# wengflow/robust-e-nerf

Hardware: AMD Instinct MI355X
Metric: train_rays_per_sec (higher is better)
Workload: dtype f32; 1 GPU; BASELINE configs[1]: synthetic ficus-like event stream, 65536 events/step/GPU = 2 renders x 65536 rays x 128 samples, arch ngp, fp32, l_diff (2 renders), fwd+bwd+Adam; sampler=uniform; sampler=uniform, samples_per_ray=128, parallelism=dp1, front_prefetched=False, mlp_precision=highest, device_counts=False, device_count_overflows=0, fwd_chunks=8, dist_world_size=1

## Files before the change

### include/ren_amd.h

```cpp
#ifndef REN_AMD_H
#define REN_AMD_H

#include <stdint.h>

#ifdef __cplusplus
extern "C" {
#endif

typedef enum ren_status {
    REN_OK = 0,
    REN_ERR_BAD_ARG = -1,
    REN_ERR_UNSUPPORTED = -2,
    REN_ERR_LAUNCH = -3
} ren_status;

enum { REN_CT_AABB = 0, REN_CT_TANH = 1, REN_CT_SPHERE = 2 };

#define REN_MAX_LEVELS 16

typedef struct ren_grid_desc {
    int32_t  n_levels;
    float    scale[REN_MAX_LEVELS];
    uint32_t res[REN_MAX_LEVELS];
    uint32_t size[REN_MAX_LEVELS];
    uint32_t offset[REN_MAX_LEVELS];
    uint32_t hashed[REN_MAX_LEVELS];
} ren_grid_desc;

typedef struct ren_scene_desc {
    float   aabb[6];
    int32_t contraction_type;
} ren_scene_desc;


int ren_abi_version(void);
enum { REN_KNOB_HGB_NO_PAIRS = 0, REN_KNOB_HGB_HALVE_REGIONS = 1, REN_KNOB_MARCH_SEQUENTIAL = 2, REN_KNOB_HG_VARIANT = 3,
       REN_KNOB_VFIELD_PLAIN = 4, REN_KNOB_HGB_SUBREGION = 5, REN_KNOB_COUNT = 6 };
int ren_set_knob(int32_t knob, int32_t value);
int ren_get_knob(int32_t knob);
const char *ren_build_info(void);

int ren_trajectory_fwd(const double *ts, int64_t B, const int64_t *tab_ts, const float *tab_pos,
                       const float *tab_quat, int64_t C, float *pos, float *rot, void *stream);
int ren_raygen_fwd(const float *Kinv, const float *px, const float *pos, const float *rot,
                   int64_t B, float *rays_o, float *rays_d, void *stream);
int ren_pose_rays_fwd(const double *ts, int64_t R, const float *px, int64_t px_rows, const float *Kinv,
                      const int64_t *tab_ts, const float *tab_pos, const float *tab_quat, int64_t C,
                      float *rays_o, float *rays_d, void *stream);

int ren_ray_aabb_intersect(const float *rays_o, const float *rays_d, int64_t n_rays,
                           const float *aabb_host, float near_plane, float far_plane,
                           float *t_min, float *t_max, void *stream);
#define REN_MARCH_VERIFIED_DIV 0x100
int ren_ray_march(const float *rays_o, const float *rays_d, const float *t_min,
                  const float *t_max, const float *jitter, int64_t n_rays,
                  const float *roi_host, const int32_t *res_host, const uint8_t *binary,
                  int32_t contraction_type, float step_size, float cone_angle,
                  int32_t mode, int32_t n_uniform,
                  const int64_t *offsets, int32_t *counts,
                  int32_t *ray_indices, float *t_starts, float *t_ends, float *interval_cache,
                  int32_t cache_cap, void *stream);

int ren_march_div_check(const float *roi, int64_t *mismatches, void *stream);
int ren_uniform(uint64_t seed, uint64_t offset, int64_t n, float *out, void *stream);
int ren_exclusive_scan(const int32_t *counts, int64_t n, int64_t *offsets, int64_t *total,
                       int64_t *scratch1024 , void *stream);

int ren_count_guard(int32_t *counts, int32_t *counts_also, int64_t n_rays, const int64_t *total, int64_t capacity,
                    int64_t *n_out, int64_t *stats, void *stream);
int ren_scan_guard(int32_t *counts, int32_t *counts_also, int64_t n_rays, int64_t *offsets, int64_t *total, int64_t capacity,
                   int64_t *n_out, int64_t *stats, int64_t *scratch1024, void *stream);
int ren_frag_zero_tail(float *feat, int64_t capacity, const int64_t *n_dev, void *stream);

int ren_visibility(const int64_t *offsets, const int32_t *counts, int64_t n_rays,
                   const float *sigmas, const float *t_starts, const float *t_ends,
                   float early_stop_eps, float alpha_thre, uint8_t *keep, int32_t *kept_counts,
                   void *stream);
int ren_compact_samples(const int64_t *offsets, const int32_t *counts, const int64_t *new_offsets,
                        int64_t n_rays, const uint8_t *keep, const float *t_starts,
                        const float *t_ends, int32_t *out_ray_indices, float *out_t_starts,
                        float *out_t_ends, void *stream);
int ren_compact_features(const int64_t *offsets, const int32_t *counts, const int64_t *new_offsets, int64_t n_rays,
                         const uint8_t *keep, const float *feat_in, float *feat_out, void *stream);
int ren_pack_info(const int32_t *ray_indices, int64_t n, int64_t n_rays, int64_t *offsets,
                  int32_t *counts, void *stream);

int ren_hashgrid_fwd(const ren_grid_desc *grid, const float *table, const float *x_unit,
                     const ren_scene_desc *scene, const float *rays_o, const float *rays_d,
                     const int32_t *ray_indices, const float *t_starts, const float *t_ends,
                     int64_t n, int32_t layout, float *feat, const int64_t *n_dev, void *stream);
int ren_hashgrid_bwd(const ren_grid_desc *grid, float *grad_table, const float *x_unit,
                     const ren_scene_desc *scene, const float *rays_o, const float *rays_d,
                     const int32_t *ray_indices, const float *t_starts, const float *t_ends,
                     int64_t n, int32_t layout, const float *dfeat, void *stream);
int ren_hashgrid_bwd_input(const ren_grid_desc *grid, const float *table, const float *x_unit,
                           const ren_scene_desc *scene, const float *rays_o, const float *rays_d,
                           const int32_t *ray_indices, const float *t_starts, const float *t_ends,
                           int64_t n, int32_t layout, const float *dfeat, float *dx, void *stream);

int64_t ren_hashgrid_bwd_binned_workspace_bytes(int64_t n);
int ren_hashgrid_bwd_binned(const ren_grid_desc *grid, float *grad_table, const float *x_unit,
                            const ren_scene_desc *scene, const float *rays_o, const float *rays_d,
                            const int32_t *ray_indices, const float *t_starts, const float *t_ends,
                            int64_t n, int32_t layout, const float *dfeat, void *workspace,
                            const int64_t *n_dev, void *stream);

int ren_mlp_fwd(const float *mlp_params, int32_t radiance_dim, int32_t activations, const float *feat,
                const ren_scene_desc *scene, const float *x_world, const float *dirs,
                const float *rays_o, const float *rays_d, const int32_t *ray_indices,
                const float *t_starts, const float *t_ends, int64_t n, int32_t density_only,
                float *rgb, float *sigma, float *base_out, void *stream);
int64_t ren_mlp_bwd_workspace_floats(int32_t radiance_dim);
int ren_mlp_bwd(const float *mlp_params, int32_t radiance_dim, int32_t activations, const float *feat,
                const float *base_out, const ren_scene_desc *scene,
                const float *x_world, const float *dirs,
                const float *rays_o, const float *rays_d, const int32_t *ray_indices,
                const float *t_starts, const float *t_ends, int64_t n,
                const float *rgb, const float *d_rgb, const float *d_sigma,
                float *d_base, float *dfeat, float *grad_mlp_params, float *workspace, void *stream);

int ren_composite_fwd(const int64_t *offsets, const int32_t *counts, int64_t n_rays,
                      const float *t_starts, const float *t_ends, const float *sigmas,
                      const float *rgbs, int32_t C, const float *bkgd,
                      float *colors, float *opacities, float *depths,
                      float *weights, float *trans, void *stream);
int ren_composite_bwd(const int64_t *offsets, const int32_t *counts, int64_t n_rays,
                      const float *t_starts, const float *t_ends, const float *sigmas,
                      const float *rgbs, int32_t C, const float *bkgd,
                      const float *weights, const float *trans, const float *opacities,
                      const float *g_colors, const float *g_opac, const float *g_depth,
                      const float *g_weights,
                      float *d_sigmas, float *d_rgbs, float *d_bkgd_per_ray, void *stream);

int ren_event_loss_fwd(const float *intensity_start, const float *intensity_end, const float *target,
                       const uint8_t *valid, int64_t B, int32_t err_fn, float *loss_sum, void *stream);
int ren_event_loss_bwd(const float *intensity_start, const float *intensity_end, const float *target,
                       const uint8_t *valid, int64_t B, int32_t err_fn, float scale,
                       const float *loss_sum, float *g_start, float *g_end, void *stream);

int ren_event_diff_loss_fwd(const float *colors, const float *opacities, const uint8_t *channel_idx, int32_t C,
                            float min_intensity, const float *target, int32_t use_validity, int64_t B, int32_t err_fn,
                            float *loss_sum, void *stream);
int ren_event_diff_loss_bwd(const float *colors, const float *opacities, const uint8_t *channel_idx, int32_t C,
                            float min_intensity, const float *target, int32_t use_validity, int64_t B, int32_t err_fn,
                            float scale, const double *scale_dev, const float *loss_sum, float *g_colors, float *intensity,
                            float *pred, uint8_t *valid, float *loss, void *stream);

int ren_event_prepare(const int64_t *start_ts, const int64_t *end_ts, const int64_t *num_pos, const int64_t *num_neg,
                      const double *u_ts_diff, const double *u_diff_start, const double *u_grad, int64_t B, float c_p,
                      float c_n, double tau, double *ts_start, double *ts_end, float *target_diff, double *ts_grad,
                      float *target_grad, double *dts_start, double *dts_end, double *dts_grad, const double *event_params,
                      void *stream);
int ren_event_param_grad(int32_t kind, int32_t err_fn, int32_t param_weight_power, const float *pred,
                         const uint8_t *valid, const int64_t *start_ts, const int64_t *end_ts, const int64_t *num_pos,
                         const int64_t *num_neg, const double *u_ts_diff, int64_t B, float c_p, float c_n,
                         float raw_ratio, double tau, float weight, float *ct_grad, double *tau_grad,
                         const double *event_params, void *stream);
int ren_event_params_refresh(const float *ct_raw, float c_n, double *tau_raw, double tau_max, double *event_params,
                             void *stream);
int ren_tau_adam_step(double *tau_raw, double *tau_grad, double *state, double tau_max, double lr, double beta1, double beta2,
                      double eps, int64_t step, double grad_scale, void *stream);

int ren_adam_step(float *param, float *grad, float *exp_avg, float *exp_avg_sq, int64_t n,
                  float lr, float beta1, float beta2, float eps, float weight_decay,
                  int64_t step, float grad_scale, int32_t zero_grad, void *stream);

#define REN_HY_STEP 0
#define REN_HY_SKIP 1
#define REN_HY_BC1 2
#define REN_HY_BC2 3
#define REN_HY_TAU_STEP 4
#define REN_HY_TAU_BC1 5
#define REN_HY_TAU_BC2 6
int ren_step_tick(double *hyper, double beta1, double beta2, const int64_t *stats_a, const int64_t *stats_b, int32_t tick_tau,
                  void *stream);
int ren_adam_step_dev(float *param, float *grad, float *exp_avg, float *exp_avg_sq, int64_t n,
                      float lr, float beta1, float beta2, float eps, float weight_decay,
                      const double *hyper, float grad_scale, int32_t zero_grad, void *stream);
int ren_tau_adam_step_dev(double *tau_raw, double *tau_grad, double *state, double tau_max, double lr, double beta1,
                          double beta2, double eps, const double *hyper, double grad_scale, void *stream);

int ren_occgrid_cell_points(const int64_t *indices, const float *jitter, int64_t m,
                            const float *roi_host, const int32_t *res_host,
                            int32_t contraction_type, float *x_world, uint8_t *valid, void *stream);
int ren_occgrid_ema(float *occs, const int64_t *indices, const uint8_t *valid, const float *sigma,
                    const float *step_sizes, float step_size, int64_t m, float ema_decay,
                    void *stream);
int ren_occgrid_ema_unique(float *occs, const int64_t *indices, const uint8_t *valid, const float *sigma,
                           const float *step_sizes, float step_size, int64_t m, float ema_decay, float *scratch_cells,
                           void *stream);
int ren_occgrid_binarize(const float *occs, int64_t cells, float occ_thre, uint8_t *binary,
                         float *scratch, void *stream);

int ren_trajectory_jvp(const double *ts, int64_t B, const int64_t *tab_ts, const float *tab_pos,
                       const float *tab_quat, int64_t C, float *pos, float *rot, float *dpos, float *drot,
                       void *stream);
int ren_raygen_jvp(const float *Kinv, const float *px, const float *pos, const float *rot, const float *dpos,
                   const float *drot, int64_t B, float *rays_o, float *rays_d, float *rays_do, float *rays_dd,
                   void *stream);
int ren_hashgrid_fwd_jvp(const ren_grid_desc *grid, const float *table, const ren_scene_desc *scene,
                         const float *rays_o, const float *rays_d, const float *rays_do, const float *rays_dd,
                         const int32_t *ray_indices, const float *t_starts, const float *t_ends, int64_t n,
                         float *feat, float *featd, const int64_t *n_dev, void *stream);
int ren_hashgrid_bwd_jvp(const ren_grid_desc *grid, float *grad_table, const ren_scene_desc *scene,
                         const float *rays_o, const float *rays_d, const float *rays_do, const float *rays_dd,
                         const int32_t *ray_indices, const float *t_starts, const float *t_ends, int64_t n,
                         const float *dfeat, const float *dfeatd, void *stream);
int ren_hashgrid_bwd_binned_jvp(const ren_grid_desc *grid, float *grad_table, const ren_scene_desc *scene,
                                const float *rays_o, const float *rays_d, const float *rays_do,
                                const float *rays_dd, const int32_t *ray_indices, const float *t_starts,
                                const float *t_ends, int64_t n, const float *dfeat, const float *dfeatd,
                                void *workspace, void *stream);
int ren_hashgrid_bwd_binned_levels(const ren_grid_desc *grid, float *grad_table, const float *x_unit,
                                   const ren_scene_desc *scene, const float *rays_o, const float *rays_d,
                                   const int32_t *ray_indices, const float *t_starts, const float *t_ends, int64_t n,
                                   int32_t layout, const float *dfeat, const float *rays_do, const float *rays_dd,
                                   const float *dfeatd, uint32_t level_mask, void *workspace, const int64_t *n_dev, void *stream);
int ren_hashgrid_bwd_binned_begin(const ren_grid_desc *grid, const float *x_unit, const ren_scene_desc *scene,
                                  const float *rays_o, const float *rays_d, const int32_t *ray_indices,
                                  const float *t_starts, const float *t_ends, int64_t n, int32_t layout,
                                  void *workspace, void *stream);
int ren_hashgrid_bwd_binned_scatter(const ren_grid_desc *grid, float *grad_table, const float *x_unit,
                                    const ren_scene_desc *scene, const float *rays_o, const float *rays_d,
                                    const int32_t *ray_indices, const float *t_starts, const float *t_ends,
                                    int64_t n, int32_t layout, const float *dfeat, int64_t first, int64_t m,
                                    void *workspace, void *stream);
int ren_hashgrid_bwd_binned_finish(const ren_grid_desc *grid, float *grad_table, int64_t n, int32_t layout,
                                   void *workspace, void *stream);
int ren_mlp_fwd_jvp(const float *mlp_params, int32_t radiance_dim, int32_t activations, const float *feat, const float *featd,
                    const ren_scene_desc *scene, const float *rays_o, const float *rays_d, const float *rays_dd,
                    const int32_t *ray_indices, const float *t_starts, const float *t_ends, int64_t n,
                    float *rgb, float *rgbd, float *sigma, float *sigmad, float *base_out, float *base_outd,
                    void *stream);
int64_t ren_mlp_bwd_jvp_workspace_floats(int32_t radiance_dim);
int ren_mlp_bwd_jvp(const float *mlp_params, int32_t radiance_dim, int32_t activations, const float *feat, const float *featd,
                    const float *base_out, const float *base_outd, const ren_scene_desc *scene,
                    const float *rays_o, const float *rays_d, const float *rays_dd, const int32_t *ray_indices,
                    const float *t_starts, const float *t_ends, int64_t n, const float *rgb,
                    const float *d_rgb, const float *d_rgbd, const float *d_sigma, const float *d_sigmad,
                    float *scratch, float *dfeat, float *dfeatd, float *grad_mlp_params, float *workspace,
                    void *stream);
int ren_mlp_fwd_jvp_x(const float *mlp_params, int32_t radiance_dim, int32_t activations, int32_t mode, const float *feat, const float *featd,
                      const ren_scene_desc *scene, const float *rays_o, const float *rays_d, const float *rays_dd,
// ... 221 lines not shown
```

### robust_e_nerf_amd/_lib.py

```python
from __future__ import annotations

import ctypes
import os
from ctypes import POINTER, Structure, c_char_p, c_double, c_float, c_int, c_int32, c_int64, c_uint32, c_void_p

HERE = os.path.dirname(os.path.abspath(__file__))
LIB_PATH = os.path.join(HERE, "csrc", "libren_amd.so")
MAX_LEVELS = 16

REN_OK, REN_ERR_BAD_ARG, REN_ERR_UNSUPPORTED, REN_ERR_LAUNCH = 0, -1, -2, -3


class RenError(RuntimeError):
    pass


class GridDesc(Structure):
    _fields_ = [("n_levels", c_int32), ("scale", c_float * MAX_LEVELS), ("res", c_uint32 * MAX_LEVELS),
                ("size", c_uint32 * MAX_LEVELS), ("offset", c_uint32 * MAX_LEVELS),
                ("hashed", c_uint32 * MAX_LEVELS)]


class SceneDesc(Structure):
    _fields_ = [("aabb", c_float * 6), ("contraction_type", c_int32)]


P = c_void_p
SIGNATURES = {
    "ren_abi_version": (c_int, []),
    "ren_build_info": (c_char_p, []),
    "ren_set_knob": (c_int, [c_int32, c_int32]),
    "ren_get_knob": (c_int, [c_int32]),
    "ren_trajectory_fwd": (c_int, [P, c_int64, P, P, P, c_int64, P, P, P]),
    "ren_raygen_fwd": (c_int, [P, P, P, P, c_int64, P, P, P]),
    "ren_pose_rays_fwd": (c_int, [P, c_int64, P, c_int64, P, P, P, P, c_int64, P, P, P]),
    "ren_ray_aabb_intersect": (c_int, [P, P, c_int64, POINTER(c_float), c_float, c_float, P, P, P]),
    "ren_march_div_check": (c_int, [POINTER(c_float), P, P]),
    "ren_ray_march": (c_int, [P, P, P, P, P, c_int64, POINTER(c_float), POINTER(c_int32), P, c_int32,
                              c_float, c_float, c_int32, c_int32, P, P, P, P, P, P, c_int32, P]),
    "ren_compact_features": (c_int, [P, P, P, c_int64, P, P, P, P]),
    "ren_uniform": (c_int, [ctypes.c_uint64, ctypes.c_uint64, c_int64, P, P]),
    "ren_exclusive_scan": (c_int, [P, c_int64, P, P, P, P]),
    "ren_count_guard": (c_int, [P, P, c_int64, P, c_int64, P, P, P]),
    "ren_scan_guard": (c_int, [P, P, c_int64, P, P, c_int64, P, P, P, P]),
    "ren_frag_zero_tail": (c_int, [P, c_int64, P, P]),
    "ren_visibility": (c_int, [P, P, c_int64, P, P, P, c_float, c_float, P, P, P]),
    "ren_compact_samples": (c_int, [P, P, P, c_int64, P, P, P, P, P, P, P]),
    "ren_pack_info": (c_int, [P, c_int64, c_int64, P, P, P]),
    "ren_hashgrid_fwd": (c_int, [POINTER(GridDesc), P, P, POINTER(SceneDesc), P, P, P, P, P, c_int64, c_int32, P, P, P]),
    "ren_hashgrid_bwd": (c_int, [POINTER(GridDesc), P, P, POINTER(SceneDesc), P, P, P, P, P, c_int64, c_int32, P, P]),
    "ren_hashgrid_bwd_input": (c_int, [POINTER(GridDesc), P, P, POINTER(SceneDesc), P, P, P, P, P, c_int64, c_int32, P, P, P]),
    "ren_hashgrid_bwd_binned_workspace_bytes": (c_int64, [c_int64]),
    "ren_hashgrid_bwd_binned": (c_int, [POINTER(GridDesc), P, P, POINTER(SceneDesc), P, P, P, P, P, c_int64, c_int32, P, P, P, P]),
    "ren_hashgrid_bwd_binned_begin": (c_int, [POINTER(GridDesc), P, POINTER(SceneDesc), P, P, P, P, P, c_int64, c_int32, P, P]),
    "ren_hashgrid_bwd_binned_scatter": (c_int, [POINTER(GridDesc), P, P, POINTER(SceneDesc), P, P, P, P, P, c_int64, c_int32, P,
                                                c_int64, c_int64, P, P]),
    "ren_hashgrid_bwd_binned_finish": (c_int, [POINTER(GridDesc), P, c_int64, c_int32, P, P]),
    "ren_mlp_fwd": (c_int, [P, c_int32, c_int32, P, POINTER(SceneDesc), P, P, P, P, P, P, P, c_int64, c_int32, P, P, P, P]),
    "ren_mlp_bwd_workspace_floats": (c_int64, [c_int32]),
    "ren_mlp_bwd": (c_int, [P, c_int32, c_int32, P, P, POINTER(SceneDesc), P, P, P, P, P, P, P, c_int64, P, P, P, P, P, P, P, P]),
    "ren_mlp_fwd_bf16": (c_int, [P, c_int32, c_int32, P, POINTER(SceneDesc), P, P, P, P, P, P, P, c_int64, c_int32, P, P, P, P]),
    "ren_mlp_bwd_bf16": (c_int, [P, c_int32, c_int32, P, P, POINTER(SceneDesc), P, P, P, P, P, P, P, c_int64, P, P, P, P, P, P, P, P]),
    "ren_mlp_act_save_floats": (c_int64, [c_int64]),
    "ren_mlp_fwd_save": (c_int, [P, c_int32, c_int32, c_int32, P, POINTER(SceneDesc), P, P, P, P, P, P, P, c_int64, P, P, P, P, P]),
    "ren_mlp_bwd_saved": (c_int, [P, c_int32, c_int32, c_int32, P, P, P, POINTER(SceneDesc), P, P, P, P, P, P, P, c_int64, P, P, P,
                                  P, P, P, P, P]),
    "ren_act_jvp_fwd": (c_int, [P, c_int32, P, c_int32, c_float, P, c_int32, c_int64, c_int32, P]),
    "ren_act_jvp_bwd": (c_int, [P, P, P, c_int32, P, c_float, P, P, c_int64, c_int32, P]),
    "ren_event_prepare": (c_int, [P, P, P, P, P, P, P, c_int64, c_float, c_float, c_double, P, P, P, P, P, P, P, P, P, P]),
    "ren_event_params_refresh": (c_int, [P, c_float, P, c_double, P, P]),
    "ren_tau_adam_step": (c_int, [P, P, P, c_double, c_double, c_double, c_double, c_double, c_int64, c_double, P]),
    "ren_event_param_grad": (c_int, [c_int32, c_int32, c_int32, P, P, P, P, P, P, P, c_int64, c_float, c_float, c_float,
                                     c_double, c_float, P, P, P, P]),
    "ren_mlp_fwd_x": (c_int, [P, c_int32, c_int32, c_int32, P, POINTER(SceneDesc), P, P, P, P, P, P, P, c_int64, c_int32, P, P, P, P, P, P]),
    "ren_mlp_bwd_x_workspace_floats": (c_int64, [c_int32]),
    "ren_mlp_bwd_x": (c_int, [P, c_int32, c_int32, c_int32, P, P, P, POINTER(SceneDesc), P, P, P, P, P, P, P, c_int64, P, P, P, P, P,
                              P, P, c_int32, P, P]),
    "ren_composite_fwd": (c_int, [P, P, c_int64, P, P, P, P, c_int32, P, P, P, P, P, P, P]),
    "ren_composite_bwd": (c_int, [P, P, c_int64, P, P, P, P, c_int32, P, P, P, P, P, P, P, P, P, P, P, P]),
    "ren_event_loss_fwd": (c_int, [P, P, P, P, c_int64, c_int32, P, P]),
    "ren_event_loss_bwd": (c_int, [P, P, P, P, c_int64, c_int32, c_float, P, P, P, P]),
    "ren_event_diff_loss_fwd": (c_int, [P, P, P, c_int32, c_float, P, c_int32, c_int64, c_int32, P, P]),
    "ren_event_diff_loss_bwd": (c_int, [P, P, P, c_int32, c_float, P, c_int32, c_int64, c_int32, c_float, P, P, P, P, P, P, P, P]),
    "ren_bkgd_param_fwd": (c_int, [P, c_int32, P, P]),
    "ren_bkgd_param_grad": (c_int, [P, c_int64, c_int32, P, P, P, P]),
    "ren_step_tick": (c_int, [P, c_double, c_double, P, P, c_int32, P]),
    "ren_adam_step_dev": (c_int, [P, P, P, P, c_int64, c_float, c_float, c_float, c_float, c_float, P, c_float, c_int32, P]),
    "ren_tau_adam_step_dev": (c_int, [P, P, P, c_double, c_double, c_double, c_double, c_double, P, c_double, P]),
    "ren_adam_step": (c_int, [P, P, P, P, c_int64, c_float, c_float, c_float, c_float, c_float, c_int64,
                              c_float, c_int32, P]),
    "ren_occgrid_cell_points": (c_int, [P, P, c_int64, POINTER(c_float), POINTER(c_int32), c_int32, P, P, P]),
    "ren_occgrid_ema": (c_int, [P, P, P, P, P, c_float, c_int64, c_float, P]),
    "ren_occgrid_ema_unique": (c_int, [P, P, P, P, P, c_float, c_int64, c_float, P, P]),
    "ren_occgrid_binarize": (c_int, [P, c_int64, c_float, P, P, P]),
    "ren_column_sum": (c_int, [P, c_int64, c_int32, P, P, P]),
    "ren_trajectory_jvp": (c_int, [P, c_int64, P, P, P, c_int64, P, P, P, P, P]),
    "ren_raygen_jvp": (c_int, [P, P, P, P, P, P, c_int64, P, P, P, P, P]),
    "ren_hashgrid_fwd_jvp": (c_int, [POINTER(GridDesc), P, POINTER(SceneDesc), P, P, P, P, P, P, P, c_int64, P, P, P, P]),
    "ren_hashgrid_bwd_jvp": (c_int, [POINTER(GridDesc), P, POINTER(SceneDesc), P, P, P, P, P, P, P, c_int64, P, P, P]),
    "ren_hashgrid_bwd_binned_jvp": (c_int, [POINTER(GridDesc), P, POINTER(SceneDesc), P, P, P, P, P, P, P, c_int64, P, P, P, P]),
    "ren_hashgrid_bwd_binned_levels": (c_int, [POINTER(GridDesc), P, P, POINTER(SceneDesc), P, P, P, P, P, c_int64, c_int32, P,
                                               P, P, P, c_uint32, P, P, P]),
    "ren_mlp_fwd_jvp": (c_int, [P, c_int32, c_int32, P, P, POINTER(SceneDesc), P, P, P, P, P, P, c_int64, P, P, P, P, P, P, P]),
    "ren_mlp_bwd_jvp_workspace_floats": (c_int64, [c_int32]),
    "ren_mlp_bwd_jvp": (c_int, [P, c_int32, c_int32, P, P, P, P, POINTER(SceneDesc), P, P, P, P, P, P, c_int64, P, P, P, P, P,
                                P, P, P, P, P, P]),
    "ren_mlp_fwd_jvp_x": (c_int, [P, c_int32, c_int32, c_int32, P, P, POINTER(SceneDesc), P, P, P, P, P, P, c_int64, P, P, P, P, P, P, P, P]),
    "ren_mlp_bwd_jvp_x_workspace_floats": (c_int64, [c_int32]),
    "ren_mlp_bwd_jvp_x": (c_int, [P, c_int32, c_int32, c_int32, P, P, P, P, POINTER(SceneDesc), P, P, P, P, P, P, c_int64, P, P, P, P, P,
                                  P, P, P, P, P, P, P]),
    "ren_composite_fwd_jvp": (c_int, [P, P, c_int64, P, P, P, P, P, P, c_int32, P, P, P, P, P, P, P, P, P]),
    "ren_composite_bwd_jvp": (c_int, [P, P, c_int64, P, P, P, P, P, P, c_int32, P, P, P, P, P, P, P, P, P, P, P, P, P, P]),
    "ren_trajectory_jvp2": (c_int, [P, c_int64, P, P, P, c_int64, P, P, P, P, P, P]),
    "ren_raygen_jvp2": (c_int, [P, P, P, P, P, P, P, c_int64, P, P, P, P, P, P]),
    "ren_hashgrid_fwd_jvp2": (c_int, [POINTER(GridDesc), P, POINTER(SceneDesc), P, P, P, P, P, P, P, P, c_int64, P, P, P, P, P]),
    "ren_mlp_fwd_jvp2": (c_int, [P, c_int32, c_int32, P, P, P, POINTER(SceneDesc), P, P, P, P, P, P, P, P, c_int64, P, P, P, P, P, P, P]),
    "ren_mlp_fwd_jvp2_x": (c_int, [P, c_int32, c_int32, c_int32, P, P, P, POINTER(SceneDesc), P, P, P, P, P, P, P, P, c_int64, P, P, P, P, P, P,
                                   P, P]),
    "ren_composite_fwd_jvp2": (c_int, [P, P, c_int64, P, P, P, P, P, P, P, P, c_int32, P, P, P, P, P]),
    "ren_freq_encode": (c_int, [POINTER(SceneDesc), P, P, P, P, P, P, P, c_int64, P, c_int32, P, c_int32, c_int32, P,
                                c_int32, c_int32, P, P]),
    "ren_dense_fwd": (c_int, [P, c_int32, P, P, c_int32, c_int32, c_int32, P, P, c_int32, c_int64, P]),
    "ren_dense_bwd_data": (c_int, [P, c_int32, P, c_int32, c_int32, c_int32, c_int32, P, c_int32, c_int32, P, c_int32,
                                   c_int64, P]),
    "ren_dense_bwd_weight_workspace_floats": (c_int64, [c_int32, c_int32, c_int32]),
    "ren_dense_bwd_weight": (c_int, [P, c_int32, P, c_int32, c_int32, c_int32, c_int64, c_int32, P, P, P, P]),
    "ren_vanilla_heads_bwd": (c_int, [P, P, P, P, c_int64, c_int32, c_int32, P, P, P]),
    "ren_vanilla_image_bytes": (c_int64, [c_int32]),
    "ren_vanilla_saved_bytes": (c_int64, [c_int32, c_int64]),
    "ren_vanilla_prep": (c_int, [P, c_int32, c_int32, P, P]),
    "ren_vanilla_fwd": (c_int, [P, c_int32, P, c_int32, P, P, c_int32, c_int32, P, c_int32, c_int64, P, P, P, P]),
    "ren_vanilla_bwd": (c_int, [P, P, P, c_int32, c_int32, c_int64, P, c_int64, P, P]),
    "ren_vanilla_bwd_weight_workspace_floats": (c_int64, [c_int32]),
    "ren_vanilla_bwd_weight": (c_int, [P, P, c_int64, P, c_int32, P, c_int32, P, P, c_int32, c_int32, c_int64, c_int32, P, P, P]),
    "ren_vanilla_bwd_weight_tangent": (c_int, [P, P, c_int64, P, c_int32, P, c_int32, P, P, c_int32, c_int32, c_int64, c_int32, P, P, P]),
    "ren_vanilla_fwd_jvp": (c_int, [P, c_int32, P, c_int32, P, P, P, P, c_int32, c_int32, P, c_int32, c_int64, P, P, P, P, P, P, P]),
    "ren_vanilla_bwd_jvp": (c_int, [P, P, P, P, P, c_int32, c_int32, c_int64, P, P, c_int64, P, P, P, P]),
    "ren_freq_encode_jvp": (c_int, [POINTER(SceneDesc), P, P, P, P, P, P, P, P, c_int64, c_int32, P, c_int32, P, c_int32, c_int32,
                                    P, c_int32, c_int32, P]),
    "ren_act_jvp2_fwd": (c_int, [P, c_int32, P, P, c_int32, c_float, P, c_int32, P, c_int32, c_int64, c_int32, P]),
    "ren_vanilla_heads_jvp": (c_int, [P, P, P, P, P, P, c_int64, c_int32, c_int32, P, P, P, P, P]),
    "ren_vanilla_heads_bwd_jvp": (c_int, [P, P, P, P, P, P, P, P, c_int64, c_int32, c_int32, P, P, P, P, P]),
    "ren_rate_epilogue": (c_int, [P, P, P, P, c_int32, c_int64, c_float, P, P, P, P, P]),
    "ren_tau_pose_grad": (c_int, [P, P, P, P, P, c_int64, P, P]),
    "ren_weight_norm_fwd": (c_int, [P, P, P, c_int32, c_int64, P, P]),
    "ren_weight_norm_bwd": (c_int, [P, P, P, P, c_int32, c_int64, P, P, c_int32, P]),
    "ren_grad_loss_fwd": (c_int, [P, P, P, P, c_int64, c_int32, P, P]),
    "ren_grad_loss_bwd": (c_int, [P, P, P, P, c_int64, c_int32, c_float, P, P, P, P, P, P]),
    "ren_ssim_scratch_doubles": (c_int64, [c_int64, c_int32, c_int32]),
    "ren_ssim_planes": (c_int, [P, P, c_int64, c_int32, c_int32, c_double, P, P, P]),
    "ren_event_frames": (c_int, [P, P, P, c_int64, P, c_int32, c_int32, c_int32, c_int32, P, P]),
    "ren_event_frame_compare_scratch_doubles": (c_int64, [c_int32, c_int32, c_int32]),
    "ren_event_frame_compare": (c_int, [P, P, P, c_int32, c_int32, c_int32, c_double, c_double, P, P, P]),
    "ren_event_intervals": (c_int, [P, P, P, c_int64, P, P, P, P]),
    "ren_event_table_write": (c_int, [P, P, P, c_int32, P, P, P, c_int64, c_int64, P, c_int32, c_int32, P, P, P, P, P, P, P, P]),
    "ren_mesh_classify": (c_int, [P, c_int32, c_int32, c_int32, c_float, P, P, P, P]),
    "ren_mesh_write": (c_int, [P, P, P, P, c_int32, c_int32, c_int32, c_float, POINTER(c_float), POINTER(c_float), POINTER(c_float),
                               c_int64, c_int64, P, P, P]),
    "ren_mesh_components": (c_int, [P, c_int32, c_int32, c_int32, c_float, c_int32, P, P, P, P]),
    "ren_mesh_component_apply": (c_int, [P, P, P, c_int64, c_float, P, P]),
    "ren_mesh_simplify_cells": (c_int, [P, c_int64, POINTER(c_double), POINTER(c_double), c_int32, c_int32, c_int32, P, P, P, P]),
    "ren_mesh_simplify_flags": (c_int, [P, c_int64, P, P]),
    "ren_mesh_simplify_faces": (c_int, [P, c_int64, c_int64, P, P, c_int64, c_int64, P, P, P, P, P]),
    "ren_mesh_simplify_heads": (c_int, [P, P, P, P, c_int64, c_int64, P, P, P]),
    "ren_mesh_simplify_vertices": (c_int, [P, P, P, P, P, c_int32, c_int32, c_int32, POINTER(c_double), POINTER(c_double), c_int64,
                                           c_int64, P, P]),
    "ren_mesh_simplify_compact_faces": (c_int, [P, P, P, P, c_int64, c_int64, c_int64, P, P]),
}

_lib = None


def load() -> ctypes.CDLL:
    global _lib
    if _lib is not None:
        return _lib
    if not os.path.exists(LIB_PATH):
        raise RenError(
            f"{LIB_PATH} is missing: build it with `python -m robust_e_nerf_amd.build` "
            "(hipcc --offload-arch=gfx950).  There is no CPU fallback.")
    from . import build as _build
    if os.environ.get("REN_ALLOW_STALE_LIB") != "1" and not _build.is_current():
        if not os.path.exists(_build.STAMP):
            import sys
            print(f"[ren_amd] warning: {_build.STAMP} is missing, cannot verify that the library matches the sources", file=sys.stderr)
        else:
            raise RenError(f"{LIB_PATH} is STALE: it was not built from the sources next to it; run "
                           "`python -m robust_e_nerf_amd.build` (or set REN_ALLOW_STALE_LIB=1 to load it anyway)")
    import torch
    lib = ctypes.CDLL(LIB_PATH)
    for name, (res, args) in SIGNATURES.items():
        try:
# ... 19 lines not shown
```

### robust_e_nerf_amd/csrc/ren_common.h

```cpp
#pragma once
#include <hip/hip_runtime.h>
#include <stdint.h>
#include <math.h>
#include <stdio.h>
#include "../../include/ren_amd.h"

#define REN_WAVE 64

#undef hipLaunchKernelGGL
#define hipLaunchKernelGGL(kernel, grid, block, shmem, stream, ...)            \
    do {                                                                        \
        (void)hipGetLastError();                                                \
        kernel<<<(grid), (block), (shmem), (stream)>>>(__VA_ARGS__);            \
    } while (0)

#define REN_CHECK_LAUNCH()                                   \
    do {                                                     \
        hipError_t e__ = hipGetLastError();                  \
        if (e__ != hipSuccess)                               \
            fprintf(stderr, "[ren_amd] %s:%d launch error: %s\n", __FILE__, __LINE__, hipGetErrorString(e__)); \
        return e__ == hipSuccess ? REN_OK : REN_ERR_LAUNCH;  \
    } while (0)

static inline int ren_blocks(int64_t n, int threads) { return (int)((n + threads - 1) / threads); }

#include <atomic>
#include <cstdlib>
inline std::atomic<int> *ren_knob_store() {
    static std::atomic<int> knobs[REN_KNOB_COUNT];
    static const bool init = [] {
        const char *names[REN_KNOB_COUNT] = {"REN_HGB_NO_PAIRS", "REN_HGB_HALVE_REGIONS", "REN_MARCH_SEQUENTIAL", "REN_HG_VARIANT",
                                           "REN_VFIELD_PLAIN", "REN_HGB_SUBREGION"};
        const int defaults[REN_KNOB_COUNT] = {0, 0, 0, 2, 0, 1};
        for (int k = 0; k < REN_KNOB_COUNT; ++k) {
            const char *e = getenv(names[k]);
            knobs[k].store(e ? atoi(e) : defaults[k], std::memory_order_relaxed);
        }
        return true;
    }();
    (void)init;
    return knobs;
}
static inline int ren_knob(int k) { return ren_knob_store()[k].load(std::memory_order_relaxed); }

struct ren_scene_dev {
    float lo[3], inv_ext[3];
    float hi[3];
    int ct;
};

static inline ren_scene_dev ren_make_scene(const ren_scene_desc *s) {
    ren_scene_dev d;
    for (int k = 0; k < 3; ++k) {
        d.lo[k] = s->aabb[k];
        d.hi[k] = s->aabb[3 + k];
        d.inv_ext[k] = 1.0f / (s->aabb[3 + k] - s->aabb[k]);
    }
    d.ct = s->contraction_type;
    return d;
}

__device__ __forceinline__ void ren_contract(const ren_scene_dev &sc, float x, float y, float z,
                                             float &ux, float &uy, float &uz) {
    ux = (x - sc.lo[0]) / (sc.hi[0] - sc.lo[0]);
    uy = (y - sc.lo[1]) / (sc.hi[1] - sc.lo[1]);
    uz = (z - sc.lo[2]) / (sc.hi[2] - sc.lo[2]);
    if (sc.ct == REN_CT_SPHERE) {
        ux = ux * 2.f - 1.f; uy = uy * 2.f - 1.f; uz = uz * 2.f - 1.f;
        float mag = sqrtf(ux * ux + uy * uy + uz * uz);
        if (mag > 1.f) {
            float s = (2.f - 1.f / mag) / mag;
            ux *= s; uy *= s; uz *= s;
        }
        ux = ux * 0.25f + 0.5f; uy = uy * 0.25f + 0.5f; uz = uz * 0.25f + 0.5f;
    } else if (sc.ct == REN_CT_TANH) {
        ux = (tanhf(ux - 0.5f) + 1.f) * 0.5f;
        uy = (tanhf(uy - 0.5f) + 1.f) * 0.5f;
        uz = (tanhf(uz - 0.5f) + 1.f) * 0.5f;
    }
}

__device__ __forceinline__ void ren_sample_pos(const float *__restrict__ rays_o,
                                               const float *__restrict__ rays_d,
                                               const int32_t *__restrict__ ray_indices,
                                               const float *__restrict__ t_starts,
                                               const float *__restrict__ t_ends, int64_t i,
                                               float &x, float &y, float &z, int &ray) {
    ray = ray_indices[i];
    float tm = (t_starts[i] + t_ends[i]) * 0.5f;
    const float *o = rays_o + 3 * (int64_t)ray, *d = rays_d + 3 * (int64_t)ray;
    x = o[0] + d[0] * tm;
    y = o[1] + d[1] * tm;
    z = o[2] + d[2] * tm;
}

__device__ __forceinline__ int64_t ren_eff_n(int64_t n, const int64_t *__restrict__ n_dev) {
    if (!n_dev) return n;
    const int64_t m = *n_dev;
    return m < n ? (m < 0 ? 0 : m) : n;
}

__device__ __forceinline__ float ren_wave_sum(float v) {
#pragma unroll
    for (int off = 32; off > 0; off >>= 1) v += __shfl_xor(v, off, 64);
    return v;
}
```

### robust_e_nerf_amd/csrc/ren_hashgrid.hip

```cpp
#include "ren_hashgrid_common.h"
#include <stdlib.h>

namespace {

__device__ __forceinline__ bool block_to_work(int xcd_affine, int n_levels, int64_t n_chunks, int &lvl,
                                              int64_t &chunk) {
    if (!xcd_affine) { lvl = blockIdx.y; chunk = blockIdx.x; return true; }
    const int64_t b = blockIdx.x;
    if (xcd_affine & 4) { lvl = (int)(b % n_levels); chunk = b / n_levels; return chunk < n_chunks; }
    const int64_t j = b >> 3;
    const int slot = (int)(j / n_chunks);
    chunk = j - slot * n_chunks;
    lvl = (int)(b & 7) + 8 * slot;
    return lvl < n_levels;
}

template <int LAYOUT, bool FROM_RAYS>
__global__ __launch_bounds__(256) void hashgrid_fwd_kernel(
    GridDev g, const float2 *__restrict__ table, const float *__restrict__ x_unit, ren_scene_dev sc,
    const float *__restrict__ rays_o, const float *__restrict__ rays_d,
    const int32_t *__restrict__ ray_indices, const float *__restrict__ t_starts,
    const float *__restrict__ t_ends, int64_t n, int64_t n_pad, float *__restrict__ feat, int xcd_affine,
    const int64_t *__restrict__ n_dev) {
    int lvl; int64_t chunk;
    if (!block_to_work(xcd_affine, g.n_levels, (n_pad + 255) / 256, lvl, chunk)) return;
    const int64_t i = chunk * blockDim.x + threadIdx.x;
    if (n_dev) {
        n = ren_eff_n(n, n_dev);
        if (LAYOUT == 1) { const int64_t p = ((n + 31) >> 5) << 5; n_pad = p < n_pad ? p : n_pad; } else n_pad = n;
    }
    if (i >= n_pad) return;
    float f0 = 0.f, f1 = 0.f;
    if (i < n) {
        float ux, uy, uz;
        if (FROM_RAYS) {
            float x, y, z; int ray;
            ren_sample_pos(rays_o, rays_d, ray_indices, t_starts, t_ends, i, x, y, z, ray);
            ren_contract(sc, x, y, z, ux, uy, uz);
        } else {
            ux = x_unit[3 * i]; uy = x_unit[3 * i + 1]; uz = x_unit[3 * i + 2];
        }
        const LevelPos p = level_pos(ux, uy, uz, g.scale[lvl]);
        const uint32_t res = g.res[lvl], size = g.size[lvl];
        const bool hashed = g.hashed[lvl] != 0;
        const float2 *tab = table + g.offset[lvl];
        float2 v[8];
        uint32_t idx[8];
        corner_indices8(p.c[0], p.c[1], p.c[2], res, size, hashed, idx);
        gather_corners8(tab, idx, v);
#pragma unroll
        for (int c = 0; c < 8; ++c) {
            const float wx = (c & 1) ? p.w[0] : 1.f - p.w[0];
            const float wy = (c & 2) ? p.w[1] : 1.f - p.w[1];
            const float wz = (c & 4) ? p.w[2] : 1.f - p.w[2];
            const float w = wx * wy * wz;
            f0 += w * v[c].x;
            f1 += w * v[c].y;
        }
    }
    if (LAYOUT == 0) {
        if (i < n) reinterpret_cast<float2 *>(feat)[i * g.n_levels + lvl] = make_float2(f0, f1);
    } else {
        const int64_t b = ((i >> 5) * REN_MAX_LEVELS + lvl) * 64 + (i & 31);
        __builtin_nontemporal_store(f0, feat + b);
        __builtin_nontemporal_store(f1, feat + b + 32);
    }
}

template <int LAYOUT, bool FROM_RAYS, bool PAIR>
__global__ __launch_bounds__(256) void hashgrid_bwd_kernel(
    GridDev g, float *__restrict__ grad_table, const float *__restrict__ x_unit, ren_scene_dev sc,
    const float *__restrict__ rays_o, const float *__restrict__ rays_d,
    const int32_t *__restrict__ ray_indices, const float *__restrict__ t_starts,
    const float *__restrict__ t_ends, int64_t n, const float *__restrict__ dfeat, int xcd_affine) {
    int lvl; int64_t chunk;
    if (PAIR) {
        if (!block_to_work(xcd_affine, g.n_levels, (n + 127) / 128, lvl, chunk)) return;
    } else {
        if (!block_to_work(xcd_affine, g.n_levels, (n + 255) / 256, lvl, chunk)) return;
    }
    const int64_t i = PAIR ? chunk * 128 + (threadIdx.x >> 1) : chunk * blockDim.x + threadIdx.x;
    const int feat_sel = PAIR ? (threadIdx.x & 1) : 0;
    if (i >= n) return;
    float d0, d1;
    if (LAYOUT == 0) {
        const float2 d = reinterpret_cast<const float2 *>(dfeat)[i * g.n_levels + lvl];
        d0 = d.x; d1 = d.y;
    } else {
        const int64_t b = ((i >> 5) * REN_MAX_LEVELS + lvl) * 64 + (i & 31);
        d0 = dfeat[b];
        d1 = dfeat[b + 32];
    }
    if (PAIR) { d0 = feat_sel ? d1 : d0; if (d0 == 0.f) return; }
    else if (d0 == 0.f && d1 == 0.f) return;
    float ux, uy, uz;
    if (FROM_RAYS) {
        float x, y, z; int ray;
        ren_sample_pos(rays_o, rays_d, ray_indices, t_starts, t_ends, i, x, y, z, ray);
        ren_contract(sc, x, y, z, ux, uy, uz);
    } else {
        ux = x_unit[3 * i]; uy = x_unit[3 * i + 1]; uz = x_unit[3 * i + 2];
    }
    const LevelPos p = level_pos(ux, uy, uz, g.scale[lvl]);
    const uint32_t res = g.res[lvl], size = g.size[lvl];
    const bool hashed = g.hashed[lvl] != 0;
    float *gt = grad_table + 2 * (size_t)g.offset[lvl];
#pragma unroll
    for (int c = 0; c < 8; ++c) {
        const uint32_t idx = corner_index(p.c[0] + (c & 1), p.c[1] + ((c >> 1) & 1), p.c[2] + (c >> 2),
                                          res, size, hashed);
        const float wx = (c & 1) ? p.w[0] : 1.f - p.w[0];
        const float wy = (c & 2) ? p.w[1] : 1.f - p.w[1];
        const float wz = (c & 4) ? p.w[2] : 1.f - p.w[2];
        const float w = wx * wy * wz;
        if (PAIR) {
            atomicAdd(gt + 2 * (size_t)idx + feat_sel, w * d0);
        } else {
            atomicAdd(gt + 2 * (size_t)idx, w * d0);
            atomicAdd(gt + 2 * (size_t)idx + 1, w * d1);
        }
    }
}

int hg_variant() { return ren_knob(REN_KNOB_HG_VARIANT); }

}

extern "C" int ren_hashgrid_fwd(const ren_grid_desc *grid, const float *table, const float *x_unit,
                                const ren_scene_desc *scene, const float *rays_o, const float *rays_d,
                                const int32_t *ray_indices, const float *t_starts, const float *t_ends,
                                int64_t n, int32_t layout, float *feat, const int64_t *n_dev, void *stream) {
    GridDev g;
    int rc = make_grid(grid, g);
    if (rc) return rc;
    if (!table || !feat || n < 0 || (layout != 0 && layout != 1)) return REN_ERR_BAD_ARG;
    const bool from_rays = x_unit == nullptr;
    if (from_rays && (!scene || !rays_o || !rays_d || !ray_indices || !t_starts || !t_ends)) return REN_ERR_BAD_ARG;
    if (layout == 1 && g.n_levels != REN_MAX_LEVELS) return REN_ERR_UNSUPPORTED;
    if (n == 0) return REN_OK;
    ren_scene_dev sc = {};
    if (scene) sc = ren_make_scene(scene);
    const int64_t n_pad = layout == 1 ? ((n + 31) / 32) * 32 : n;
    const int variant = hg_variant();
    const int affine = variant & 5;
    const int64_t n_chunks = (n_pad + 255) / 256;
    dim3 grd = (affine & 4) ? dim3((unsigned)(g.n_levels * n_chunks))
             : affine ? dim3((unsigned)(8 * ((g.n_levels + 7) / 8) * n_chunks)) : dim3((unsigned)n_chunks, g.n_levels);
    dim3 blk(256);
    const float2 *tab = reinterpret_cast<const float2 *>(table);
#define LAUNCH(L, R)                                                                                     \
    hipLaunchKernelGGL((hashgrid_fwd_kernel<L, R>), grd, blk, 0, (hipStream_t)stream, g, tab, x_unit, sc, \
                       rays_o, rays_d, ray_indices, t_starts, t_ends, n, n_pad, feat, affine, n_dev)
    if (layout == 0) { if (from_rays) LAUNCH(0, true); else LAUNCH(0, false); }
    else             { if (from_rays) LAUNCH(1, true); else LAUNCH(1, false); }
#undef LAUNCH
    REN_CHECK_LAUNCH();
}

extern "C" int ren_hashgrid_bwd(const ren_grid_desc *grid, float *grad_table, const float *x_unit,
                                const ren_scene_desc *scene, const float *rays_o, const float *rays_d,
                                const int32_t *ray_indices, const float *t_starts, const float *t_ends,
                                int64_t n, int32_t layout, const float *dfeat, void *stream) {
    GridDev g;
    int rc = make_grid(grid, g);
    if (rc) return rc;
    if (!grad_table || !dfeat || n < 0 || (layout != 0 && layout != 1)) return REN_ERR_BAD_ARG;
    const bool from_rays = x_unit == nullptr;
    if (from_rays && (!scene || !rays_o || !rays_d || !ray_indices || !t_starts || !t_ends)) return REN_ERR_BAD_ARG;
    if (layout == 1 && g.n_levels != REN_MAX_LEVELS) return REN_ERR_UNSUPPORTED;
    if (n == 0) return REN_OK;
    ren_scene_dev sc = {};
    if (scene) sc = ren_make_scene(scene);
    const int variant = hg_variant();
    const int affine = variant & 1;
    const bool pair = (variant & 2) != 0;
    const int64_t n_chunks = pair ? (n + 127) / 128 : (n + 255) / 256;
    dim3 grd = affine ? dim3((unsigned)(8 * ((g.n_levels + 7) / 8) * n_chunks)) : dim3((unsigned)n_chunks, g.n_levels);
    dim3 blk(256);
#define LAUNCH(L, R, P)                                                                                          \
    hipLaunchKernelGGL((hashgrid_bwd_kernel<L, R, P>), grd, blk, 0, (hipStream_t)stream, g, grad_table, x_unit, \
                       sc, rays_o, rays_d, ray_indices, t_starts, t_ends, n, dfeat, affine)
#define LAUNCH2(L, R) do { if (pair) LAUNCH(L, R, true); else LAUNCH(L, R, false); } while (0)
    if (layout == 0) { if (from_rays) LAUNCH2(0, true); else LAUNCH2(0, false); }
    else             { if (from_rays) LAUNCH2(1, true); else LAUNCH2(1, false); }
#undef LAUNCH2
#undef LAUNCH
    REN_CHECK_LAUNCH();
}
```

### robust_e_nerf_amd/csrc/ren_sampling.hip

```cpp
#include "ren_common.h"
#include <cstdlib>

namespace {

struct MarchArgs {
    float roi[6];
    int res[3];
    int type;
    float step_size, cone_angle;
    int mode, n_uniform;
    float rinv[3];
    float rext[3];
    int fastdiv;
};

__device__ __forceinline__ float clampf(float v, float lo, float hi) { return v < lo ? lo : (v > hi ? hi : v); }

__global__ void ray_aabb_kernel(const float *__restrict__ o, const float *__restrict__ d, int64_t n,
                                float a0, float a1, float a2, float a3, float a4, float a5,
                                float near_plane, float far_plane,
                                float *__restrict__ t_min, float *__restrict__ t_max) {
    int64_t i = (int64_t)blockIdx.x * blockDim.x + threadIdx.x;
    if (i >= n) return;
    const float *ro = o + 3 * i, *rd = d + 3 * i;
    float tmin = (a0 - ro[0]) / rd[0], tmax = (a3 - ro[0]) / rd[0];
    if (tmin > tmax) { float t = tmin; tmin = tmax; tmax = t; }
    float tymin = (a1 - ro[1]) / rd[1], tymax = (a4 - ro[1]) / rd[1];
    if (tymin > tymax) { float t = tymin; tymin = tymax; tymax = t; }
    bool miss = (tmin > tymax) || (tymin > tmax);
    if (!miss) {
        if (tymin > tmin) tmin = tymin;
        if (tymax < tmax) tmax = tymax;
        float tzmin = (a2 - ro[2]) / rd[2], tzmax = (a5 - ro[2]) / rd[2];
        if (tzmin > tzmax) { float t = tzmin; tzmin = tzmax; tzmax = t; }
        miss = (tmin > tzmax) || (tzmin > tmax);
        if (!miss) {
            if (tzmin > tmin) tmin = tzmin;
            if (tzmax < tmax) tmax = tzmax;
        }
    }
    float lo, hi;
    if (miss) { lo = 1e10f; hi = 1e10f; }
    else { lo = tmin > 0.f ? tmin : 0.f; hi = tmax; }
    if (near_plane == near_plane) lo = lo < near_plane ? near_plane : lo;
    if (far_plane == far_plane) hi = hi > far_plane ? far_plane : hi;
    t_min[i] = lo;
    t_max[i] = hi;
}

__device__ __forceinline__ float div_verified(float a, float b, float y) {
    const float q0 = a * y;
    return __fmaf_rn(__fmaf_rn(-q0, b, a), y, q0);
}
__device__ __forceinline__ void roi_to_unit(const float *p, const MarchArgs &a, float *u) {
    float num[3];
#pragma unroll
    for (int k = 0; k < 3; ++k) num[k] = p[k] - a.roi[k];
    if (a.fastdiv) {
#pragma unroll
        for (int k = 0; k < 3; ++k) u[k] = div_verified(num[k], a.roi[3 + k] - a.roi[k], a.rext[k]);
        return;
    }
#pragma unroll
    for (int k = 0; k < 3; ++k) u[k] = num[k] / (a.roi[3 + k] - a.roi[k]);
}

__device__ __forceinline__ bool grid_occupied_at(const float *p, const float *u0, const MarchArgs &a,
                                                 const uint8_t *__restrict__ binary) {
    if (a.type == REN_CT_AABB) {
#pragma unroll
        for (int k = 0; k < 3; ++k)
            if (p[k] < a.roi[k] || p[k] > a.roi[3 + k]) return false;
    }
    float u[3] = {u0[0], u0[1], u0[2]};
    if (a.type == REN_CT_SPHERE) {
#pragma unroll
        for (int k = 0; k < 3; ++k) u[k] = u[k] * 2.f - 1.f;
        float norm = sqrtf(u[0] * u[0] + u[1] * u[1] + u[2] * u[2]);
        if (norm > 1.f) {
            float s = (2.f - 1.f / norm);
#pragma unroll
            for (int k = 0; k < 3; ++k) u[k] = s * (u[k] / norm);
        }
#pragma unroll
        for (int k = 0; k < 3; ++k) u[k] = u[k] * 0.25f + 0.5f;
    } else if (a.type == REN_CT_TANH) {
#pragma unroll
        for (int k = 0; k < 3; ++k) u[k] = tanhf(u[k] - 0.5f) * 0.5f + 0.5f;
    }
    int idx = 0;
#pragma unroll
    for (int k = 0; k < 3; ++k) {
        int c = (int)(u[k] * (float)a.res[k]);
        c = c < 0 ? 0 : (c > a.res[k] - 1 ? a.res[k] - 1 : c);
        idx = idx * a.res[k] + c;
    }
    return binary[idx] != 0;
}

__device__ __forceinline__ float sgnf(float v) { return (float)((v > 0.f) - (v < 0.f)); }

__device__ __forceinline__ float distance_to_next_voxel(const float *u, const float *dir,
                                                        const float *inv_dir, const MarchArgs &a) {
    float t = 1e30f;
#pragma unroll
    for (int k = 0; k < 3; ++k) {
        float r = (float)a.res[k];
        float x = u[k] * r;
        const float q = (floorf(x + 0.5f + 0.5f * sgnf(dir[k])) - x) * inv_dir[k];
        float tx = (a.rinv[k] != 0.f ? q * a.rinv[k] : q / r) * (a.roi[3 + k] - a.roi[k]);
        if (tx < t) t = tx;
    }
    return t > 0.f ? t : 0.f;
}

__device__ __forceinline__ float calc_dt(float t, float cone_angle, float dt_min, float dt_max) {
    return clampf(t * cone_angle, dt_min, dt_max);
}

template <bool WRITE>
__global__ void ray_march_kernel(const float *__restrict__ o, const float *__restrict__ d,
                                 const float *__restrict__ t_min, const float *__restrict__ t_max,
                                 const float *__restrict__ jitter, int64_t n_rays, MarchArgs a,
                                 const uint8_t *__restrict__ binary,
                                 const int64_t *__restrict__ offsets, int32_t *__restrict__ counts,
                                 int32_t *__restrict__ ray_indices, float *__restrict__ t_starts,
                                 float *__restrict__ t_ends, float2 *__restrict__ cache, int cache_cap) {
    int64_t i = (int64_t)blockIdx.x * blockDim.x + threadIdx.x;
    if (i >= n_rays) return;
    if (WRITE && cache && counts[i] <= cache_cap) return;
    if (WRITE && counts && counts[i] == 0) return;
    const float ro[3] = {o[3 * i], o[3 * i + 1], o[3 * i + 2]};
    const float rd[3] = {d[3 * i], d[3 * i + 1], d[3 * i + 2]};
    float near = t_min[i];
    const float far = t_max[i];
    const int64_t base = WRITE ? offsets[i] : 0;
    int j = 0;
    if (a.mode == 1) {
        if (near < far) {
            float delta = (far - near) / (float)a.n_uniform;
            float first = jitter ? near + jitter[i] * delta : near;
            if (WRITE) {
                for (j = 0; j < a.n_uniform; ++j) {
                    float t0 = first + (float)j * delta;
                    t_starts[base + j] = t0;
                    t_ends[base + j] = t0 + delta;
                    ray_indices[base + j] = (int32_t)i;
                }
            }
            j = a.n_uniform;
        }
        if (!WRITE) counts[i] = j;
        return;
    }
    if (jitter) near = near + jitter[i] * a.step_size;
    const float inv_dir[3] = {1.f / rd[0], 1.f / rd[1], 1.f / rd[2]};
    const float dt_min = a.step_size, dt_max = 1e10f;
    float t0 = near;
    float dt = calc_dt(t0, a.cone_angle, dt_min, dt_max);
    float t1 = t0 + dt;
    float t_mid = (t0 + t1) * 0.5f;
    while (t_mid < far) {
        float p[3] = {ro[0] + t_mid * rd[0], ro[1] + t_mid * rd[1], ro[2] + t_mid * rd[2]}, u[3];
        roi_to_unit(p, a, u);
        if (grid_occupied_at(p, u, a, binary)) {
            if (WRITE) {
                t_starts[base + j] = t0;
                t_ends[base + j] = t1;
                ray_indices[base + j] = (int32_t)i;
            } else if (cache && j < cache_cap) {
                cache[i * cache_cap + j] = make_float2(t0, t1);
            }
            ++j;
            t0 = t1;
            t1 = t0 + calc_dt(t0, a.cone_angle, dt_min, dt_max);
            t_mid = (t0 + t1) * 0.5f;
        } else if (a.type == REN_CT_AABB) {
            float t_target = t_mid + distance_to_next_voxel(u, rd, inv_dir, a);
            do { t_mid += dt_min; } while (t_mid < t_target);
            dt = calc_dt(t_mid, a.cone_angle, dt_min, dt_max);
            t0 = t_mid - dt * 0.5f;
            t1 = t_mid + dt * 0.5f;
        } else {
            t0 = t1;
            t1 = t0 + calc_dt(t0, a.cone_angle, dt_min, dt_max);
            t_mid = (t0 + t1) * 0.5f;
        }
    }
    if (!WRITE) counts[i] = j;
}

template <bool WRITE, int SPEC>
__global__ __launch_bounds__(256) void ray_march_spec_kernel(
    const float *__restrict__ o, const float *__restrict__ d, const float *__restrict__ t_min,
    const float *__restrict__ t_max, const float *__restrict__ jitter, int64_t n_rays, MarchArgs a,
    const uint8_t *__restrict__ binary, const int64_t *__restrict__ offsets, int32_t *__restrict__ counts,
    int32_t *__restrict__ ray_indices, float *__restrict__ t_starts, float *__restrict__ t_ends,
    float2 *__restrict__ cache, int cache_cap) {
    const int64_t i = ((int64_t)blockIdx.x * blockDim.x + threadIdx.x) / SPEC;
    const int l = threadIdx.x % SPEC, lane = threadIdx.x & 63, g0 = lane - l;
    bool done = i >= n_rays;
    if (!done && WRITE && cache && counts[i] <= cache_cap) done = true;
    if (!done && WRITE && counts && counts[i] == 0) done = true;
    float ro[3] = {0.f, 0.f, 0.f}, rd[3] = {1.f, 1.f, 1.f};
    float near = 0.f, far = 0.f;
    int64_t base = 0;
    if (!done) {
#pragma unroll
        for (int k = 0; k < 3; ++k) { ro[k] = o[3 * i + k]; rd[k] = d[3 * i + k]; }
        near = t_min[i]; far = t_max[i];
        if (WRITE) base = offsets[i];
        if (jitter) near = near + jitter[i] * a.step_size;
    }
    const float inv_dir[3] = {1.f / rd[0], 1.f / rd[1], 1.f / rd[2]};
    const float dt_min = a.step_size, dt_max = 1e10f;
    float t0 = near;
    float t1 = t0 + calc_dt(t0, a.cone_angle, dt_min, dt_max);
    float t_mid = (t0 + t1) * 0.5f;
    int j = 0;
    const bool is_aabb = a.type == REN_CT_AABB;
    if (!(t_mid < far)) done = true;
    auto empty_step = [&](float tm, float &n0, float &n1, float &nm) {
        const float p[3] = {ro[0] + tm * rd[0], ro[1] + tm * rd[1], ro[2] + tm * rd[2]};
        float u[3];
        roi_to_unit(p, a, u);
        const float t_target = tm + distance_to_next_voxel(u, rd, inv_dir, a);
        do { tm += dt_min; } while (tm < t_target);
        const float dt = calc_dt(tm, a.cone_angle, dt_min, dt_max);
        n0 = tm - dt * 0.5f;
        n1 = tm + dt * 0.5f;
        nm = tm;
    };
    bool emode = false;
    while (__any(!done)) {
        if (emode) {
            float e0 = t0, e1 = t1, em = t_mid;
#pragma unroll 1
            for (int k = 0; k < SPEC - 1; ++k)
                if (k < l && !done && em < far) empty_step(em, e0, e1, em);
            const bool in = !done && em < far;
            bool occ = false;
            if (in) {
                const float p[3] = {ro[0] + em * rd[0], ro[1] + em * rd[1], ro[2] + em * rd[2]};
                float u[3];
                roi_to_unit(p, a, u);
                occ = grid_occupied_at(p, u, a, binary);
            }
            const unsigned in_bits = (unsigned)(__ballot(in) >> g0) & ((1u << SPEC) - 1u);
            const unsigned occ_bits = (unsigned)(__ballot(occ) >> g0) & ((1u << SPEC) - 1u);
            const int e = __builtin_ctz((occ_bits | ~in_bits) | (1u << SPEC));
            const int src = g0 + (e < SPEC ? e : SPEC - 1);
            const float b0 = __shfl(e0, src, 64), b1 = __shfl(e1, src, 64), bm = __shfl(em, src, 64);
            if (!done) {
                if (e == SPEC) {
                    empty_step(bm, t0, t1, t_mid);
                } else {
                    t0 = b0; t1 = b1; t_mid = bm;
                    emode = false;
                }
                if (!(t_mid < far)) done = true;
            }
            continue;
        }
        float a0 = t0, a1 = t1, am = t_mid;
#pragma unroll
        for (int k = 0; k < SPEC - 1; ++k)
            if (k < l) { a0 = a1; a1 = a0 + calc_dt(a0, a.cone_angle, dt_min, dt_max); am = (a0 + a1) * 0.5f; }
        const bool in = !done && am < far;
        bool occ = false;
        if (in) {
            const float p[3] = {ro[0] + am * rd[0], ro[1] + am * rd[1], ro[2] + am * rd[2]};
            float u[3];
            roi_to_unit(p, a, u);
            occ = grid_occupied_at(p, u, a, binary);
        }
        const unsigned in_bits = (unsigned)(__ballot(in) >> g0) & ((1u << SPEC) - 1u);
        const unsigned occ_bits = (unsigned)(__ballot(occ) >> g0) & ((1u << SPEC) - 1u);
        const int n_in = __builtin_ctz(~in_bits | (1u << SPEC));
        const int f = is_aabb ? __builtin_ctz(~occ_bits | (1u << SPEC)) : n_in;
        const bool emit = !done && l < f && occ;
        if (emit) {
            const int at = j + __popc(occ_bits & ((1u << l) - 1u));
            if (WRITE) {
                t_starts[base + at] = a0;
                t_ends[base + at] = a1;
                ray_indices[base + at] = (int32_t)i;
            } else if (cache && at < cache_cap) {
                cache[i * cache_cap + at] = make_float2(a0, a1);
            }
        }
        const int src = g0 + (f < SPEC ? f : SPEC - 1);
        const float b0 = __shfl(a0, src, 64), b1 = __shfl(a1, src, 64), bm = __shfl(am, src, 64);
        if (!done) {
            j += __popc(occ_bits & ((1u << f) - 1u));
            if (f == SPEC) {
                t0 = b1;
                t1 = t0 + calc_dt(t0, a.cone_angle, dt_min, dt_max);
                t_mid = (t0 + t1) * 0.5f;
            } else if (f >= n_in) {
                done = true;
            } else {
                empty_step(bm, t0, t1, t_mid);
                emode = true;
            }
            if (!(t_mid < far)) done = true;
        }
    }
    if (!WRITE && l == 0 && i < n_rays) counts[i] = j;
}

__global__ __launch_bounds__(256) void cached_write_kernel(const float2 *__restrict__ cache, int cache_cap, int64_t n_rays,
                                                           const int64_t *__restrict__ offsets,
                                                           const int32_t *__restrict__ counts,
                                                           int32_t *__restrict__ ray_indices, float *__restrict__ t_starts,
                                                           float *__restrict__ t_ends) {
    const int64_t g = (int64_t)blockIdx.x * blockDim.x + threadIdx.x;
    const int64_t i = g >> 3;
    if (i >= n_rays) return;
    const int c = counts[i];
    if (c > cache_cap) return;
    const int64_t base = offsets[i];
    const float2 *src = cache + i * cache_cap;
    for (int j = (int)(g & 7); j < c; j += 8) {
        const float2 v = src[j];
        t_starts[base + j] = v.x;
        t_ends[base + j] = v.y;
        ray_indices[base + j] = (int32_t)i;
    }
}

__global__ __launch_bounds__(256) void uniform_write_kernel(const float *__restrict__ t_min, const float *__restrict__ t_max,
                                                            const float *__restrict__ jitter, int64_t n_rays, int n_uniform,
                                                            const int64_t *__restrict__ offsets,
                                                            int32_t *__restrict__ ray_indices, float *__restrict__ t_starts,
                                                            float *__restrict__ t_ends) {
    const int64_t g = (int64_t)blockIdx.x * blockDim.x + threadIdx.x;
    const int64_t i = g / n_uniform;
    const int j = (int)(g - i * n_uniform);
    if (i >= n_rays) return;
    const float near = t_min[i], far = t_max[i];
    if (!(near < far)) return;
    const float delta = (far - near) / (float)n_uniform;
    const float first = jitter ? near + jitter[i] * delta : near;
    const float t0 = first + (float)j * delta;
    const int64_t at = offsets[i] + j;
    t_starts[at] = t0;
    t_ends[at] = t0 + delta;
    ray_indices[at] = (int32_t)i;
}

constexpr int SCAN_TILE = 1024;

__global__ __launch_bounds__(1024) void scan_tiles_kernel(const int32_t *__restrict__ counts, int64_t n,
                                                          int64_t *__restrict__ offsets) {
    __shared__ int64_t wsum[16];
    const int tid = threadIdx.x, lane = tid & 63, wave = tid >> 6;
    const int64_t i = (int64_t)blockIdx.x * SCAN_TILE + tid;
    const int64_t c = i < n ? counts[i] : 0;
    int64_t v = c;
#pragma unroll
    for (int off = 1; off < 64; off <<= 1) {
        const int64_t t = __shfl_up(v, off, 64);
        if (lane >= off) v += t;
    }
    if (lane == 63) wsum[wave] = v;
    __syncthreads();
    int64_t base = 0;
    for (int w = 0; w < wave; ++w) base += wsum[w];
    if (i < n) offsets[i] = base + v - c;
}

__global__ __launch_bounds__(1024) void scan_sums_kernel(const int32_t *__restrict__ counts, int64_t n, int n_tiles,
                                                         const int64_t *__restrict__ offsets,
                                                         int64_t *__restrict__ tile_base, int64_t *__restrict__ total) {
    __shared__ int64_t part[1024];
    const int tid = threadIdx.x;
    int64_t s = 0;
    if (tid < n_tiles) {
        const int64_t last = ((int64_t)tid + 1) * SCAN_TILE - 1 < n ? ((int64_t)tid + 1) * SCAN_TILE - 1 : n - 1;
        s = offsets[last] + counts[last];
    }
    part[tid] = s;
    __syncthreads();
    for (int off = 1; off < 1024; off <<= 1) {
        const int64_t v = tid >= off ? part[tid - off] : 0;
        __syncthreads();
        part[tid] += v;
        __syncthreads();
    }
    if (tid < n_tiles) tile_base[tid] = part[tid] - s;
    if (tid == 1023 && total) total[0] = part[1023];
}

__global__ __launch_bounds__(1024) void scan_add_kernel(int64_t n, const int64_t *__restrict__ tile_base,
                                                        int64_t *__restrict__ offsets) {
    const int64_t i = (int64_t)blockIdx.x * SCAN_TILE + threadIdx.x;
    if (i < n) offsets[i] += tile_base[blockIdx.x];
}

__global__ __launch_bounds__(1024) void exclusive_scan_kernel(const int32_t *__restrict__ counts, int64_t n,
                                                              int64_t *__restrict__ offsets,
                                                              int64_t *__restrict__ total) {
    __shared__ int64_t part[1024];
    const int tid = threadIdx.x;
    const int64_t per = (n + 1023) / 1024;
    const int64_t b = tid * per, e = (b + per < n) ? b + per : n;
    int64_t s = 0;
    for (int64_t i = b; i < e; ++i) s += counts[i];
    part[tid] = s;
    __syncthreads();
    for (int off = 1; off < 1024; off <<= 1) {
        int64_t v = tid >= off ? part[tid - off] : 0;
        __syncthreads();
        part[tid] += v;
        __syncthreads();
    }
    int64_t run = part[tid] - s;
    for (int64_t i = b; i < e; ++i) { offsets[i] = run; run += counts[i]; }
    if (tid == 1023 && total) total[0] = part[1023];
}

__global__ __launch_bounds__(256) void visibility_kernel(const int64_t *__restrict__ offsets, const int32_t *__restrict__ counts,
                                  int64_t n_rays, const float *__restrict__ sigmas,
                                  const float *__restrict__ t_starts, const float *__restrict__ t_ends,
                                  float eps, float alpha_thre, uint8_t *__restrict__ keep,
                                  int32_t *__restrict__ kept_counts) {
    const int64_t i = ((int64_t)blockIdx.x * blockDim.x + threadIdx.x) >> 6;
    const int lane = threadIdx.x & 63;
    if (i >= n_rays) return;
    const int64_t b = offsets[i];
    const int cnt = counts[i];
    float T = 1.f;
    int kept = 0;
    for (int c0 = 0; c0 < cnt; c0 += 64) {
        const bool valid = c0 + lane < cnt;
        const int64_t j = b + c0 + lane;
        float alpha = 0.f;
        if (valid) alpha = 1.f - expf(-sigmas[j] * (t_ends[j] - t_starts[j]));
        const float om = 1.f - alpha;
        float t_here = 0.f;
#pragma unroll
        for (int l = 0; l < 64; ++l) {
            if (lane == l) t_here = T;
            T = T * __builtin_bit_cast(float, __builtin_amdgcn_readlane(__builtin_bit_cast(int, om), l));
        }
        bool k = valid && t_here >= eps;
        if (alpha_thre > 0.f) k = k && (alpha >= alpha_thre);
        if (valid) keep[j] = (uint8_t)k;
        kept += __popcll(__ballot(k));
    }
    if (lane == 0) kept_counts[i] = kept;
}

__global__ __launch_bounds__(256) void compact_kernel(const int64_t *__restrict__ offsets, const int32_t *__restrict__ counts,
                               const int64_t *__restrict__ new_offsets, int64_t n_rays,
                               const uint8_t *__restrict__ keep, const float *__restrict__ t_starts,
                               const float *__restrict__ t_ends, int32_t *__restrict__ out_ri,
                               float *__restrict__ out_ts, float *__restrict__ out_te) {
    const int64_t i = ((int64_t)blockIdx.x * blockDim.x + threadIdx.x) >> 6;
    const int lane = threadIdx.x & 63;
    if (i >= n_rays) return;
    const int64_t b = offsets[i];
    const int cnt = counts[i];
    int64_t w = new_offsets[i];
    for (int c0 = 0; c0 < cnt; c0 += 64) {
        const bool valid = c0 + lane < cnt;
        const int64_t j = b + c0 + lane;
        const bool k = valid && keep[j];
        const unsigned long long m = __ballot(k);
        if (k) {
            const int64_t at = w + __popcll(m & ((1ull << lane) - 1ull));
            out_ri[at] = (int32_t)i;
            out_ts[at] = t_starts[j];
            out_te[at] = t_ends[j];
        }
        w += __popcll(m);
    }
}

__global__ __launch_bounds__(256) void compact_features_kernel(const int64_t *__restrict__ offsets, const int32_t *__restrict__ counts,
                                        const int64_t *__restrict__ new_offsets, int64_t n_rays,
                                        const uint8_t *__restrict__ keep, const float *__restrict__ feat_in,
                                        float *__restrict__ feat_out) {
    const int64_t i = ((int64_t)blockIdx.x * blockDim.x + threadIdx.x) >> 6;
    const int lane = threadIdx.x & 63;
    if (i >= n_rays) return;
    const int64_t b = offsets[i];
    const int cnt = counts[i];
    int64_t w = new_offsets[i];
    for (int c0 = 0; c0 < cnt; c0 += 64) {
        const bool valid = c0 + lane < cnt;
        const int64_t j = b + c0 + lane;
        const bool k = valid && keep[j];
        const unsigned long long m = __ballot(k);
        if (k) {
            const int64_t at = w + __popcll(m & ((1ull << lane) - 1ull));
            const float *src = feat_in + (j >> 5) * 1024 + (j & 31);
            float *dst = feat_out + (at >> 5) * 1024 + (at & 31);
            float v[32];
#pragma unroll
            for (int q = 0; q < 32; ++q) v[q] = src[q * 32];
#pragma unroll
            for (int q = 0; q < 32; ++q) dst[q * 32] = v[q];
        }
        w += __popcll(m);
    }
}

__global__ void zero_i32_kernel(int32_t *p, int64_t n) {
    int64_t i = (int64_t)blockIdx.x * blockDim.x + threadIdx.x;
    if (i < n) p[i] = 0;
}

__global__ void pack_info_kernel(const int32_t *__restrict__ ri, int64_t n, int64_t *__restrict__ offsets,
                                 int32_t *__restrict__ counts) {
    int64_t i = (int64_t)blockIdx.x * blockDim.x + threadIdx.x;
    if (i >= n) return;
    const int32_t r = ri[i];
    if (i == 0 || ri[i - 1] != r) {
        offsets[r] = i;
    }
    if (i == n - 1 || ri[i + 1] != r) {
        int64_t s = i;
        while (s > 0 && ri[s - 1] == r) --s;
        counts[r] = (int32_t)(i + 1 - s);
    }
}

__global__ void fill_empty_offsets_kernel(int64_t *offsets, const int32_t *counts, int64_t n_rays) {
    int64_t i = (int64_t)blockIdx.x * blockDim.x + threadIdx.x;
    if (i < n_rays && counts[i] == 0) offsets[i] = 0;
}

}

extern "C" int ren_ray_aabb_intersect(const float *rays_o, const float *rays_d, int64_t n_rays,
                                      const float *aabb, float near_plane, float far_plane,
                                      float *t_min, float *t_max, void *stream) {
    if (!rays_o || !rays_d || !aabb || !t_min || !t_max || n_rays < 0) return REN_ERR_BAD_ARG;
    if (n_rays == 0) return REN_OK;
    hipLaunchKernelGGL(ray_aabb_kernel, dim3(ren_blocks(n_rays, 256)), dim3(256), 0, (hipStream_t)stream,
                       rays_o, rays_d, n_rays, aabb[0], aabb[1], aabb[2], aabb[3], aabb[4], aabb[5],
                       near_plane, far_plane, t_min, t_max);
    REN_CHECK_LAUNCH();
}

__global__ __launch_bounds__(256) void march_div_check_kernel(float b0, float b1, float b2, float y0, float y1, float y2,
                                                              unsigned long long *__restrict__ mismatches) {
    const float b[3] = {b0, b1, b2}, y[3] = {y0, y1, y2};
    unsigned bad = 0;
    const uint32_t t = blockIdx.x * blockDim.x + threadIdx.x;
    const uint32_t low = (t & 0x7fffffu) | ((t >> 23) << 31);
    for (uint32_t e = 27; e <= 226; ++e) {
        const float a = __uint_as_float(low | (e << 23));
#pragma unroll
        for (int k = 0; k < 3; ++k) {
            const float q = a / b[k], f = div_verified(a, b[k], y[k]);
            bad += __float_as_uint(q) != __float_as_uint(f);
        }
    }
    if (bad) atomicAdd(mismatches, (unsigned long long)bad);
}

extern "C" int ren_march_div_check(const float *roi, int64_t *mismatches, void *stream) {
    if (!roi || !mismatches) return REN_ERR_BAD_ARG;
    float b[3], y[3];
    for (int k = 0; k < 3; ++k) {
        b[k] = roi[3 + k] - roi[k];
        if (!(b[k] > 0x1p-60f) || !(b[k] < 0x1p60f)) return REN_ERR_BAD_ARG;
        if (!(fabsf(roi[k]) >= 0x1p-60f) || !(fabsf(roi[k]) < 0x1p60f)) return REN_ERR_UNSUPPORTED;
        y[k] = 1.f / b[k];
    }
    (void)hipMemsetAsync(mismatches, 0, sizeof(int64_t), (hipStream_t)stream);
    hipLaunchKernelGGL(march_div_check_kernel, dim3(1 << 16), dim3(256), 0, (hipStream_t)stream, b[0], b[1], b[2], y[0], y[1], y[2],
                       reinterpret_cast<unsigned long long *>(mismatches));
    REN_CHECK_LAUNCH();
}

extern "C" int ren_ray_march(const float *rays_o, const float *rays_d, const float *t_min,
                             const float *t_max, const float *jitter, int64_t n_rays,
                             const float *roi, const int32_t *res, const uint8_t *binary,
                             int32_t contraction_type, float step_size, float cone_angle,
                             int32_t mode, int32_t n_uniform, const int64_t *offsets, int32_t *counts,
                             int32_t *ray_indices, float *t_starts, float *t_ends, float *interval_cache,
                             int32_t cache_cap, void *stream) {
    if (!rays_o || !rays_d || !t_min || !t_max || n_rays < 0) return REN_ERR_BAD_ARG;
    const bool verified_div = (mode & REN_MARCH_VERIFIED_DIV) != 0;
    mode &= ~REN_MARCH_VERIFIED_DIV;
    if (mode != 0 && mode != 1) return REN_ERR_BAD_ARG;
    if (mode == 0 && (!roi || !res || !binary || step_size <= 0.f)) return REN_ERR_BAD_ARG;
    if (mode == 1 && n_uniform <= 0) return REN_ERR_BAD_ARG;
    if (contraction_type < 0 || contraction_type > 2) return REN_ERR_BAD_ARG;
    const bool write = t_starts != nullptr;
    if (write && (!offsets || !t_ends || !ray_indices)) return REN_ERR_BAD_ARG;
    if (!write && !counts) return REN_ERR_BAD_ARG;
    if (interval_cache && (cache_cap <= 0 || !counts)) return REN_ERR_BAD_ARG;
    if (n_rays == 0) return REN_OK;
    float2 *cache = mode == 0 ? reinterpret_cast<float2 *>(interval_cache) : nullptr;
    MarchArgs a;
    for (int k = 0; k < 6; ++k) a.roi[k] = roi ? roi[k] : (k < 3 ? -1e10f : 1e10f);
    for (int k = 0; k < 3; ++k) a.res[k] = res ? res[k] : 1;
    for (int k = 0; k < 3; ++k) a.rinv[k] = (a.res[k] > 0 && (a.res[k] & (a.res[k] - 1)) == 0) ? 1.f / (float)a.res[k] : 0.f;
    a.type = contraction_type; a.step_size = step_size; a.cone_angle = cone_angle;
    a.mode = mode; a.n_uniform = n_uniform;
    for (int k = 0; k < 3; ++k) a.rext[k] = 1.f / (a.roi[3 + k] - a.roi[k]);
    a.fastdiv = verified_div && roi ? 1 : 0;
    dim3 grid(ren_blocks(n_rays, 64)), block(64);
    const int kn = ren_knob(REN_KNOB_MARCH_SEQUENTIAL);
    int width = n_rays <= 10240 ? 16 : n_rays <= 24576 ? 8 : n_rays <= 81920 ? 4 : 0;
    if (kn == 1) width = 0;
    else if (kn == 2 || kn == 4 || kn == 8 || kn == 16) width = kn;
    if (mode != 0) width = 0;
    const dim3 sgrid(ren_blocks(n_rays * (width ? width : 1), 256));
#define REN_MARCH_SPEC(WRITE)                                                                                              \
    do {                                                                                                                   \
        if (width == 16)                                                                                                   \
            hipLaunchKernelGGL((ray_march_spec_kernel<WRITE, 16>), sgrid, dim3(256), 0, (hipStream_t)stream, rays_o, rays_d, \
                               t_min, t_max, jitter, n_rays, a, binary, offsets, counts, ray_indices, t_starts, t_ends,    \
                               cache, cache_cap);                                                                          \
        else if (width == 8)                                                                                               \
            hipLaunchKernelGGL((ray_march_spec_kernel<WRITE, 8>), sgrid, dim3(256), 0, (hipStream_t)stream, rays_o, rays_d, \
                               t_min, t_max, jitter, n_rays, a, binary, offsets, counts, ray_indices, t_starts, t_ends,    \
                               cache, cache_cap);                                                                          \
        else if (width == 4)                                                                                               \
            hipLaunchKernelGGL((ray_march_spec_kernel<WRITE, 4>), sgrid, dim3(256), 0, (hipStream_t)stream, rays_o, rays_d, \
                               t_min, t_max, jitter, n_rays, a, binary, offsets, counts, ray_indices, t_starts, t_ends,    \
                               cache, cache_cap);                                                                          \
        else                                                                                                               \
            hipLaunchKernelGGL((ray_march_spec_kernel<WRITE, 2>), sgrid, dim3(256), 0, (hipStream_t)stream, rays_o, rays_d, \
                               t_min, t_max, jitter, n_rays, a, binary, offsets, counts, ray_indices, t_starts, t_ends,    \
                               cache, cache_cap);                                                                          \
    } while (0)
    if (write && mode == 1)
        hipLaunchKernelGGL(uniform_write_kernel, dim3(ren_blocks(n_rays * n_uniform, 256)), dim3(256), 0,
                           (hipStream_t)stream, t_min, t_max, jitter, n_rays, n_uniform, offsets, ray_indices,
                           t_starts, t_ends);
    else if (write) {
        if (cache)
            hipLaunchKernelGGL(cached_write_kernel, dim3(ren_blocks(n_rays * 8, 256)), dim3(256), 0, (hipStream_t)stream,
                               cache, cache_cap, n_rays, offsets, counts, ray_indices, t_starts, t_ends);
        if (width)
            REN_MARCH_SPEC(true);
        else
            hipLaunchKernelGGL(ray_march_kernel<true>, grid, block, 0, (hipStream_t)stream, rays_o, rays_d,
                               t_min, t_max, jitter, n_rays, a, binary, offsets, counts, ray_indices,
                               t_starts, t_ends, cache, cache_cap);
    } else if (width)
        REN_MARCH_SPEC(false);
    else
        hipLaunchKernelGGL(ray_march_kernel<false>, grid, block, 0, (hipStream_t)stream, rays_o, rays_d,
                           t_min, t_max, jitter, n_rays, a, binary, offsets, counts, ray_indices,
                           t_starts, t_ends, cache, cache_cap);
#undef REN_MARCH_SPEC
    REN_CHECK_LAUNCH();
}

__global__ __launch_bounds__(256) void philox_uniform_kernel(uint64_t seed, uint64_t offset, int64_t n, float *__restrict__ out) {
    const int64_t g = (int64_t)blockIdx.x * blockDim.x + threadIdx.x;
    if (4 * g >= n) return;
    uint32_t c[4] = {(uint32_t)g, (uint32_t)((uint64_t)g >> 32), (uint32_t)offset, (uint32_t)(offset >> 32)};
    uint32_t k0 = (uint32_t)seed, k1 = (uint32_t)(seed >> 32);
#pragma unroll
    for (int r = 0; r < 10; ++r) {
        const uint64_t p0 = (uint64_t)0xD2511F53u * c[0], p1 = (uint64_t)0xCD9E8D57u * c[2];
        const uint32_t n0 = (uint32_t)(p1 >> 32) ^ c[1] ^ k0, n2 = (uint32_t)(p0 >> 32) ^ c[3] ^ k1;
        c[1] = (uint32_t)p1; c[3] = (uint32_t)p0; c[0] = n0; c[2] = n2;
        k0 += 0x9E3779B9u; k1 += 0xBB67AE85u;
    }
#pragma unroll
    for (int j = 0; j < 4; ++j)
        if (4 * g + j < n) out[4 * g + j] = (float)(c[j] >> 8) * 5.9604644775390625e-8f;
}

extern "C" int ren_uniform(uint64_t seed, uint64_t offset, int64_t n, float *out, void *stream) {
    if (!out || n < 0) return REN_ERR_BAD_ARG;
    if (n == 0) return REN_OK;
    hipLaunchKernelGGL(philox_uniform_kernel, dim3(ren_blocks((n + 3) / 4, 256)), dim3(256), 0, (hipStream_t)stream, seed, offset, n, out);
    REN_CHECK_LAUNCH();
}

constexpr int SCAN_ONE = 65536;
__global__ __launch_bounds__(1024) void scan_guard_kernel(int32_t *__restrict__ counts, int32_t *__restrict__ counts_also, int64_t n,
                                                          int seg, int64_t *__restrict__ offsets, int64_t *__restrict__ total,
                                                          int guard, int64_t capacity, int64_t *__restrict__ n_out,
                                                          int64_t *__restrict__ stats) {
    __shared__ int64_t wsum[17];
    const int tid = threadIdx.x, lane = tid & 63, wave = tid >> 6;
    const int64_t w0 = (int64_t)wave * seg;
    auto load4 = [&](int64_t at) {
        int4 v = make_int4(0, 0, 0, 0);
        if (at + 3 < n) v = *reinterpret_cast<const int4 *>(counts + at);
        else if (at < n) {
            v.x = counts[at];
            if (at + 1 < n) v.y = counts[at + 1];
            if (at + 2 < n) v.z = counts[at + 2];
        }
        return v;
    };
    int64_t s = 0;
    for (int k = lane * 4; k < seg; k += 256) {
        const int4 v = load4(w0 + k);
        s += (int64_t)v.x + v.y + v.z + v.w;
    }
#pragma unroll
    for (int off = 32; off > 0; off >>= 1) s += __shfl_xor(s, off, 64);
    if (lane == 0) wsum[wave] = s;
    __syncthreads();
    if (tid == 0) {
        int64_t acc = 0;
        for (int w = 0; w < 16; ++w) { const int64_t t = wsum[w]; wsum[w] = acc; acc += t; }
        wsum[16] = acc;
    }
    __syncthreads();
    int64_t carry = wsum[wave];
    const int64_t tot = wsum[16];
    for (int k = lane * 4; k < seg; k += 256) {
        const int64_t at = w0 + k;
        const int4 v = load4(at);
        const int64_t t = (int64_t)v.x + v.y + v.z + v.w;
        int64_t inc = t;
#pragma unroll
        for (int off = 1; off < 64; off <<= 1) {
            const int64_t u = __shfl_up(inc, off, 64);
            if (lane >= off) inc += u;
        }
        const int64_t o0 = carry + inc - t, o1 = o0 + v.x, o2 = o1 + v.y, o3 = o2 + v.z;
        if (at + 3 < n) {
            *reinterpret_cast<longlong2 *>(offsets + at) = make_longlong2(o0, o1);
            *reinterpret_cast<longlong2 *>(offsets + at + 2) = make_longlong2(o2, o3);
        } else if (at < n) {
            offsets[at] = o0;
            if (at + 1 < n) offsets[at + 1] = o1;
            if (at + 2 < n) offsets[at + 2] = o2;
        }
        carry += __shfl(inc, 63, 64);
    }
    if (tid == 0 && total) total[0] = tot;
    if (!guard) return;
    const bool over = tot > capacity;
    if (tid == 0) {
        n_out[0] = over ? 0 : tot;
        if (stats) { stats[0] = tot; stats[1] = over ? 1 : 0; }
    }
    if (over) {
        __syncthreads();
        for (int64_t k = tid; k < n; k += 1024) {
            counts[k] = 0;
            if (counts_also) counts_also[k] = 0;
        }
    }
}

static bool scan_one_launch(int32_t *counts, int32_t *counts_also, int64_t n, int64_t *offsets, int64_t *total, int guard,
                            int64_t capacity, int64_t *n_out, int64_t *stats, hipStream_t st) {
    if (n > SCAN_ONE || n < 1 || ((uintptr_t)counts & 15) || ((uintptr_t)offsets & 15)) return false;
    int seg = (int)((n + 15) / 16);
    seg = (seg + 255) & ~255;
    hipLaunchKernelGGL(scan_guard_kernel, dim3(1), dim3(1024), 0, st, counts, counts_also, n, seg, offsets, total, guard, capacity,
                       n_out, stats);
    return true;
}

extern "C" int ren_exclusive_scan(const int32_t *counts, int64_t n, int64_t *offsets, int64_t *total,
                                  int64_t *scratch1024, void *stream) {
    if (!counts || !offsets || n < 0) return REN_ERR_BAD_ARG;
    hipStream_t st = (hipStream_t)stream;
    if (scan_one_launch(const_cast<int32_t *>(counts), nullptr, n, offsets, total, 0, 0, nullptr, nullptr, st)) { REN_CHECK_LAUNCH(); }
    const int64_t n_tiles = (n + SCAN_TILE - 1) / SCAN_TILE;
    if (scratch1024 && n_tiles >= 2 && n_tiles <= 1024) {
        hipLaunchKernelGGL(scan_tiles_kernel, dim3((unsigned)n_tiles), dim3(SCAN_TILE), 0, st, counts, n, offsets);
        hipLaunchKernelGGL(scan_sums_kernel, dim3(1), dim3(1024), 0, st, counts, n, (int)n_tiles, offsets, scratch1024, total);
        hipLaunchKernelGGL(scan_add_kernel, dim3((unsigned)n_tiles), dim3(SCAN_TILE), 0, st, n, scratch1024, offsets);
    } else {
        hipLaunchKernelGGL(exclusive_scan_kernel, dim3(1), dim3(1024), 0, st, counts, n, offsets, total);
    }
    REN_CHECK_LAUNCH();
}

__global__ __launch_bounds__(256) void count_guard_kernel(int32_t *__restrict__ counts, int32_t *__restrict__ counts_also,
                                                          int64_t n_rays, const int64_t *__restrict__ total, int64_t capacity,
                                                          int64_t *__restrict__ n_out, int64_t *__restrict__ stats) {
    const int64_t t = total[0];
    const bool over = t > capacity;
    const int64_t r = (int64_t)blockIdx.x * blockDim.x + threadIdx.x;
    if (over && r < n_rays) {
        counts[r] = 0;
        if (counts_also) counts_also[r] = 0;
    }
    if (r == 0) {
        n_out[0] = over ? 0 : t;
        if (stats) { stats[0] = t; stats[1] = over ? 1 : 0; }
    }
}

extern "C" int ren_count_guard(int32_t *counts, int32_t *counts_also, int64_t n_rays, const int64_t *total, int64_t capacity,
                               int64_t *n_out, int64_t *stats, void *stream) {
    if (!counts || !total || !n_out || n_rays < 0 || capacity < 0) return REN_ERR_BAD_ARG;
    hipLaunchKernelGGL(count_guard_kernel, dim3(ren_blocks(n_rays > 0 ? n_rays : 1, 256)), dim3(256), 0, (hipStream_t)stream,
                       counts, counts_also, n_rays, total, capacity, n_out, stats);
    REN_CHECK_LAUNCH();
}

extern "C" int ren_scan_guard(int32_t *counts, int32_t *counts_also, int64_t n_rays, int64_t *offsets, int64_t *total,
                              int64_t capacity, int64_t *n_out, int64_t *stats, int64_t *scratch1024, void *stream) {
    if (!counts || !offsets || !total || !n_out || n_rays < 0 || capacity < 0) return REN_ERR_BAD_ARG;
    if (scan_one_launch(counts, counts_also, n_rays, offsets, total, 1, capacity, n_out, stats, (hipStream_t)stream)) { REN_CHECK_LAUNCH(); }
    const int rc = ren_exclusive_scan(counts, n_rays, offsets, total, scratch1024, stream);
    if (rc != REN_OK) return rc;
    return ren_count_guard(counts, counts_also, n_rays, total, capacity, n_out, stats, stream);
}

__global__ __launch_bounds__(64) void frag_zero_tail_kernel(float *__restrict__ feat, int64_t capacity, const int64_t *__restrict__ n_dev) {
    const int64_t n = ren_eff_n(capacity, n_dev);
    const int lane = threadIdx.x & 31, half = threadIdx.x >> 5;
    if ((n & 31) == 0 || lane < (n & 31)) return;
    float *b = feat + (n >> 5) * (int64_t)(REN_MAX_LEVELS * 64) + lane;
    for (int l = 0; l < REN_MAX_LEVELS; ++l) b[l * 64 + half * 32] = 0.f;
}

extern "C" int ren_frag_zero_tail(float *feat, int64_t capacity, const int64_t *n_dev, void *stream) {
    if (!feat || !n_dev || capacity < 0) return REN_ERR_BAD_ARG;
    if (capacity == 0) return REN_OK;
    hipLaunchKernelGGL(frag_zero_tail_kernel, dim3(1), dim3(64), 0, (hipStream_t)stream, feat, capacity, n_dev);
    REN_CHECK_LAUNCH();
}

extern "C" int ren_visibility(const int64_t *offsets, const int32_t *counts, int64_t n_rays,
                              const float *sigmas, const float *t_starts, const float *t_ends,
                              float early_stop_eps, float alpha_thre, uint8_t *keep,
                              int32_t *kept_counts, void *stream) {
    if (!offsets || !counts || !sigmas || !t_starts || !t_ends || !keep || !kept_counts || n_rays < 0)
        return REN_ERR_BAD_ARG;
    if (n_rays == 0) return REN_OK;
    hipLaunchKernelGGL(visibility_kernel, dim3(ren_blocks(n_rays * 64, 256)), dim3(256), 0, (hipStream_t)stream,
                       offsets, counts, n_rays, sigmas, t_starts, t_ends, early_stop_eps, alpha_thre, keep,
                       kept_counts);
    REN_CHECK_LAUNCH();
}

extern "C" int ren_compact_samples(const int64_t *offsets, const int32_t *counts,
                                   const int64_t *new_offsets, int64_t n_rays, const uint8_t *keep,
                                   const float *t_starts, const float *t_ends,
                                   int32_t *out_ray_indices, float *out_t_starts, float *out_t_ends,
                                   void *stream) {
    if (!offsets || !counts || !new_offsets || !keep || !t_starts || !t_ends || !out_ray_indices ||
        !out_t_starts || !out_t_ends || n_rays < 0)
        return REN_ERR_BAD_ARG;
    if (n_rays == 0) return REN_OK;
    hipLaunchKernelGGL(compact_kernel, dim3(ren_blocks(n_rays * 64, 256)), dim3(256), 0, (hipStream_t)stream,
                       offsets, counts, new_offsets, n_rays, keep, t_starts, t_ends, out_ray_indices,
                       out_t_starts, out_t_ends);
    REN_CHECK_LAUNCH();
}

extern "C" int ren_compact_features(const int64_t *offsets, const int32_t *counts, const int64_t *new_offsets,
                                    int64_t n_rays, const uint8_t *keep, const float *feat_in, float *feat_out,
                                    void *stream) {
    if (!offsets || !counts || !new_offsets || !keep || !feat_in || !feat_out || n_rays < 0) return REN_ERR_BAD_ARG;
    if (n_rays == 0) return REN_OK;
    hipLaunchKernelGGL(compact_features_kernel, dim3(ren_blocks(n_rays * 64, 256)), dim3(256), 0, (hipStream_t)stream,
                       offsets, counts, new_offsets, n_rays, keep, feat_in, feat_out);
    REN_CHECK_LAUNCH();
}

extern "C" int ren_pack_info(const int32_t *ray_indices, int64_t n, int64_t n_rays, int64_t *offsets,
                             int32_t *counts, void *stream) {
    if (!offsets || !counts || n < 0 || n_rays < 0 || (n > 0 && !ray_indices)) return REN_ERR_BAD_ARG;
    if (n_rays == 0) return REN_OK;
    hipLaunchKernelGGL(zero_i32_kernel, dim3(ren_blocks(n_rays, 256)), dim3(256), 0, (hipStream_t)stream,
                       counts, n_rays);
    if (n > 0)
        hipLaunchKernelGGL(pack_info_kernel, dim3(ren_blocks(n, 256)), dim3(256), 0, (hipStream_t)stream,
                           ray_indices, n, offsets, counts);
    hipLaunchKernelGGL(fill_empty_offsets_kernel, dim3(ren_blocks(n_rays, 256)), dim3(256), 0,
                       (hipStream_t)stream, offsets, counts, n_rays);
    REN_CHECK_LAUNCH();
}
```

### robust_e_nerf_amd/engine.py

```python
from __future__ import annotations

import math
from dataclasses import dataclass, field as dc_field
from typing import Dict, Optional, Sequence, Tuple

import dataclasses
import os
import threading
import torch

from . import ops
from .fronts import DiffFront, GradFront, StepFronts
from .sample_counts import CountLog, SampleCounts, device_words
from .step_graph import StepGraphs


@dataclass
class RenderCfg:
    aabb: Tuple[float, ...] = (-1.5, -1.5, -1.5, 1.5, 1.5, 1.5)
    contraction_type: int = ops.AABB
    occ_res: Tuple[int, int, int] = (128, 128, 128)
    near_plane: Optional[float] = None
    far_plane: Optional[float] = None
    render_step_size: float = math.sqrt(3) * 3.0 / 1024
    cone_angle: float = 0.0
    early_stop_eps: float = 1e-4
    alpha_thre: float = 0.0
    min_modeled_intensity: float = 1e-3
    opacity_eps: float = 1e-10
    radiance_dim: int = 1
    sampler: str = "occgrid"
    n_uniform: int = 128
    occ_thre: float = 1e-2
    ema_decay: float = 0.95
    warmup_steps: int = 256
    occ_n: int = 16
    occ_seed: int = 20230
    binned_scatter: bool = True
    mlp_kernels: str = "x"
    save_activations: Optional[bool] = None
    march_cache: int = 512
    fwd_chunks: int = 8
    bwd_chunks: int = 1
    bwd_mlp_cus: int = 192
    dp_overlap: bool = True
    dp_split_level: int = 8
    dp_compress: Optional[str] = None
    device_counts: Optional[bool] = None
    mlp_bf16: bool = False
    mlp_precision: str = "highest"
    base_hidden_activation: str = "softplus"
    density_activation: str = "shifted_trunc_exp"
    head_hidden_activation: str = "softplus"
    radiance_activation: str = "softplus"


class NGPField:

    WN_WEIGHTS = ("base.w0", "base.wo", "head.w0", "head.w1", "head.wo")

    def __init__(self, device, radiance_dim: int = 1, pos_encoding: Optional[dict] = None,
                 weight_norm: Tuple[bool, bool] = (False, False)):
        pe = dict(n_levels=16, n_features_per_level=2, log2_hashmap_size=19, base_resolution=16,
                  per_level_scale=1.4472692012786865, otype="HashGrid")
        if pos_encoding:
            pe.update({k: v for k, v in pos_encoding.items() if k in pe})
        self.grid, self.n_table = ops.make_grid_desc(**pe)
        if self.grid.n_levels != 16:
            raise NotImplementedError("the fused MLP kernels are built for 16 levels x 2 features")
        self.C = radiance_dim
        self.n_mlp = ops.mlp_param_count(radiance_dim)
        self.weight_norm = (bool(weight_norm[0]), bool(weight_norm[1]))
        sl = ops.mlp_slices(radiance_dim)
        self.wn_layers, layers, n_g = [], [], 0
        for k in self.WN_WEIGHTS:
            if self.weight_norm[0 if k.startswith("base") else 1]:
                off, (rows, cols) = sl[k]
                self.wn_layers.append((k, n_g, rows))
                layers.append((off, rows, cols, n_g))
                n_g += rows
        self.n_wn_g = n_g
        n = self.n_table + self.n_mlp + n_g
        self.n_params = n
        n_pad = (n + 3) // 4 * 4
        self.flat = torch.zeros(n_pad, device=device, dtype=torch.float32)
        from .parallel import AUX_FLOATS
        self.grad_all = torch.zeros(n_pad + AUX_FLOATS, device=device, dtype=torch.float32)
        self.grad = self.grad_all[:n_pad]
        self.aux = self.grad_all[n_pad:]
        self.table = self.flat[: self.n_table]
        self.g_table = self.grad[: self.n_table]
        m0, m1 = self.n_table, self.n_table + self.n_mlp
        if n_g == 0:
            self.mlp, self.g_mlp = self.flat[m0: m1], self.grad[m0: m1]
        else:
            self.mlp_raw, self.wn_g = self.flat[m0: m1], self.flat[m1: n]
            self.g_mlp_raw, self.g_wn_g = self.grad[m0: m1], self.grad[m1: n]
            self.mlp = torch.zeros(self.n_mlp, device=device, dtype=torch.float32)
            self.g_mlp = torch.zeros(self.n_mlp, device=device, dtype=torch.float32)
            self._wn_table = ops.weight_norm_layers(layers)

    def refresh(self):
        if self.n_wn_g:
            ops.weight_norm_fwd(self.mlp_raw, self.wn_g, self._wn_table, self.mlp)

    def fold_grads(self, zero: bool = True):
        if self.n_wn_g:
            ops.weight_norm_bwd(self.mlp_raw, self.wn_g, self.g_mlp, self._wn_table, self.g_mlp_raw, self.g_wn_g, zero_d_eff=zero)

    def load(self, p: Dict[str, torch.Tensor]):
        dev = self.flat.device
        self.table.copy_(p["hash"].to(dev, torch.float32).reshape(-1))
        raw = self.mlp_raw if self.n_wn_g else self.mlp
        g_of = {k: (g0, rows) for k, g0, rows in self.wn_layers}
        for k, (off, shape) in ops.mlp_slices(self.C).items():
            if k in g_of:
                g0, rows = g_of[k]
                v = (p[k + "_v"] if k + "_v" in p else p[k]).to(dev, torch.float32)
                g = p[k + "_g"].to(dev, torch.float32).reshape(-1) if k + "_g" in p else v.norm(dim=1)
                raw[off: off + math.prod(shape)].copy_(v.reshape(-1))
                self.wn_g[g0: g0 + rows].copy_(g)
            else:
                if k + "_v" in p:
                    raise ValueError(f"{k}: weight_g / weight_v given for an MLP built without weight_norm")
                raw[off: off + math.prod(shape)].copy_(p[k].to(dev, torch.float32).reshape(-1))
        self.refresh()

    def mlp_views(self, grad: bool = False) -> Dict[str, torch.Tensor]:
        buf = self.g_mlp if grad else self.mlp
        return {k: buf[off: off + math.prod(shape)].view(shape) for k, (off, shape) in ops.mlp_slices(self.C).items()}

    def trainable_views(self, grad: bool = False) -> Dict[str, torch.Tensor]:
        if not self.n_wn_g:
            return self.mlp_views(grad)
        raw, gg = (self.g_mlp_raw, self.g_wn_g) if grad else (self.mlp_raw, self.wn_g)
        g_of = {k: (g0, rows) for k, g0, rows in self.wn_layers}
        out = {}
        for k, (off, shape) in ops.mlp_slices(self.C).items():
            view = raw[off: off + math.prod(shape)].view(shape)
            if k in g_of:
                g0, rows = g_of[k]
                out[k + "_g"], out[k + "_v"] = gg[g0: g0 + rows].view(rows, 1), view
            else:
                out[k] = view
        return out


@dataclass
class Packed:
    ray_indices: torch.Tensor
    t_starts: torch.Tensor
    t_ends: torch.Tensor
    offsets: torch.Tensor
    counts: torch.Tensor
    n: int
    n_marched: int = 0
    feat: Optional[torch.Tensor] = None
    n_dev: Optional[torch.Tensor] = None
    log: Optional["CountLog"] = None


def pack_batch(batch: Dict[str, torch.Tensor]) -> Dict[str, torch.Tensor]:
    items = [(k, v) for k, v in batch.items() if isinstance(v, torch.Tensor) and k != "_pack"]
    offs, total = [], 0
    for _, v in items:
        offs.append(total)
        total += (v.numel() * v.element_size() + 15) // 16 * 16
    dev = items[0][1].device
    buf = torch.empty(max(total, 16), dtype=torch.uint8, device=dev)
    out = {k: v for k, v in batch.items() if not isinstance(v, torch.Tensor)}
    for (k, v), o in zip(items, offs):
        view = buf[o: o + v.numel() * v.element_size()].view(v.dtype).view(v.shape)
        view.copy_(v)
        out[k] = view
    out["_pack"] = buf
    return out


_PINNED = threading.local()


def _host_int(t: torch.Tensor) -> int:
    cur = torch.cuda.current_stream(t.device)
    if cur == torch.cuda.default_stream(t.device):
        return int(t.item())
    bufs = _PINNED.__dict__.setdefault("bufs", {})
    buf = bufs.get(t.dtype)
    if buf is None:
        buf = bufs[t.dtype] = torch.empty(1, dtype=t.dtype).pin_memory()
    buf.copy_(t.reshape(1), non_blocking=True)
    ev = torch.cuda.Event()
    ev.record(cur)
    ev.synchronize()
    return int(buf[0])


class Renderer:
    def __init__(self, fld: NGPField, cfg: RenderCfg):
        self.field = fld
        self.cfg = cfg = dataclasses.replace(cfg)
        if os.environ.get("REN_MARCH_CACHE"):
            cfg.march_cache = int(os.environ["REN_MARCH_CACHE"])
        self.scene = ops.make_scene_desc(cfg.aabb, cfg.contraction_type)
        dev = fld.flat.device
        cells = cfg.occ_res[0] * cfg.occ_res[1] * cfg.occ_res[2]
        self.occs = torch.zeros(cells, device=dev, dtype=torch.float32)
        self.binary = torch.zeros(cells, device=dev, dtype=torch.uint8)
        self._scratch = torch.zeros(4, device=dev, dtype=torch.float32)
        self._ws = torch.empty(max(ops.mlp_bwd_workspace_floats(fld.C), ops.mlp_bwd_x_workspace_floats(fld.C)),
                               device=dev, dtype=torch.float32)
        self._bin_ws, self._bin_ws_small = None, 0
        self._normal_scratch = None
        self._occ_scratch = None
        self._occ_gen = None
        self.grad_sync = None
        self._fwd_streams = None
        self._bwd_stream = None
        self._reuse_prepass_feat = True
        self._march_div_ok = None
        self.counts = SampleCounts()
        self._capture = None
        self.dp_early_enabled = True
        self.bwd_side_cus = 0
        self._act_code = ops.activation_code(cfg.base_hidden_activation, cfg.density_activation, cfg.head_hidden_activation,
                                             cfg.radiance_activation)
        if cfg.mlp_precision not in ("highest", "high", "medium"):
            raise ValueError(f"mlp_precision {cfg.mlp_precision!r}: highest | high | medium")
        if cfg.mlp_precision == "medium":
            cfg.mlp_bf16 = True
        if self._act_code != 0 and isinstance(fld, NGPField):
            cfg.mlp_kernels = "f32"
        grid = getattr(fld, "grid", None)
        if grid is not None and not ops.binned_supported(grid):
            cfg.binned_scatter = False

    def sample_begin(self, o, d, jitter: Optional[torch.Tensor], training: bool, device_counts=False) -> dict:
        return self._scan_counts(self._march_count(o, d, jitter, training), device_counts)

    def sample_begin_merged(self, rays, training: bool, device_counts=False):
        jit = None if any(r[2] is None for r in rays) else torch.cat([r[2] for r in rays])
        st = self._march_count(torch.cat([r[0] for r in rays]), torch.cat([r[1] for r in rays]), jit, training)
        out, a = [], 0
        for o, _, _ in rays:
            b = a + o.shape[0]
            args = tuple(v[a:b] if (k < 5 and v is not None) else v for k, v in enumerate(st["args"]))
            out.append(self._scan_counts(dict(args=args, cache=None if st["cache"] is None else st["cache"][a:b],
                                              counts=st["counts"][a:b], mode=st["mode"]), device_counts))
            a = b
        return out

    def _march_count(self, o, d, jitter, training: bool) -> dict:
        c = self.cfg
        scene_aabb = c.aabb if c.contraction_type == ops.AABB else None
        if scene_aabb is not None:
            t_min, t_max = ops.ray_aabb_intersect(o, d, scene_aabb, c.near_plane, c.far_plane)
        else:
            if c.near_plane is not None and c.far_plane is not None:
                if c.near_plane < 0:
                    raise ValueError("near_plane < 0")
                t_min, t_max = ops.ray_aabb_intersect(o, d, (-1e30,) * 3 + (1e30,) * 3, c.near_plane, c.far_plane)
            else:
                n = o.shape[0]
                t_min = torch.full((n,), 0.0 if c.near_plane is None else c.near_plane, device=o.device)
                t_max = torch.full((n,), 1e10 if c.far_plane is None else c.far_plane, device=o.device)
        mode = 0 if c.sampler == "occgrid" else 1
        if mode == 0 and o.is_cuda:
            if self._march_div_ok is None:
                self._march_div_ok = ops.march_div_check(c.aabb, o.device)
        march_mode = mode | (ops.MARCH_VERIFIED_DIV if (mode == 0 and self._march_div_ok) else 0)
        jit = jitter if training else None
        args = (o, d, t_min, t_max, jit, c.aabb, c.occ_res, self.binary, c.contraction_type,
                c.render_step_size, c.cone_angle, march_mode, c.n_uniform)
        cache = torch.empty(o.shape[0], c.march_cache, 2, device=o.device) if (mode == 0 and c.march_cache > 0) else None
        counts = ops.ray_march_count(*args, cache=cache)
        return dict(args=args, cache=cache, counts=counts, mode=mode)

    def _scan_counts(self, st: dict, device_counts) -> dict:
        counts, mode, n_rays = st["counts"], st["mode"], st["counts"].shape[0]
        dcst = None
        caps = self.counts.capacities(n_rays) if (device_counts is True and mode == 0 and self.device_counts_ok()) else None
        if caps is not None:
            stats, nd = device_words(counts.device)
            offsets, total = ops.scan_guard(counts, caps[0], nd[0:1], stats[0:2])
            dcst = dict(caps=caps, stats=stats, nd=nd)
        else:
            offsets, total = ops.exclusive_scan(counts)
        return dict(st, offsets=offsets, total=total, dc=dcst)

    _spr = property(lambda self: self.counts.spr, lambda self, v: setattr(self.counts, "spr", v))

    def device_counts_ok(self) -> bool:
        c = self.cfg
        return (c.device_counts is not False and c.sampler == "occgrid" and type(self) is Renderer and c.mlp_kernels == "x" and
                c.binned_scatter and self.field.flat.is_cuda)

    def _sample_device_counts(self, o, d, st, caps, keep_feat: bool) -> Packed:
        c = self.cfg
        args, cache, counts, offsets = st["args"], st["cache"], st["counts"], st["offsets"]
        if st.get("dc") is not None:
            caps, stats, nd = st["dc"]["caps"], st["dc"]["stats"], st["dc"]["nd"]
        else:
            stats, nd = device_words(o.device)
            ops.count_guard(counts, st["total"], caps[0], nd[0:1], stats[0:2])
        cap0, cap1 = caps
        n0_dev, n1_dev = nd[0:1], nd[1:2]
        ri, ts, te = ops.ray_march_write(*args, offsets, cap0, counts=counts, cache=cache)
        keep_feat = keep_feat and self._reuse_prepass_feat
        sigma = self._density_stream(o, d, (ri, ts, te), cap0, keep_feat, n_dev=n0_dev)
        feat0 = None
        if keep_feat:
            sigma, feat0 = sigma
        keep, kept = ops.visibility(offsets, counts, sigma, ts, te, c.early_stop_eps, c.alpha_thre)
        new_offsets, total2 = ops.scan_guard(kept, cap1, n1_dev, stats[2:4], counts_also=counts)
        ri2, ts2, te2 = ops.compact_samples(offsets, counts, new_offsets, keep, ts, te, cap1)
        feat1 = ops.compact_features(offsets, counts, new_offsets, keep, feat0, cap1, n_dev=n1_dev) if feat0 is not None else None
        log = self.counts.log(o.shape[0], caps, stats, self._capture)
        return Packed(ri2, ts2, te2, new_offsets, kept, cap1, cap0, feat1, n_dev=n1_dev, log=log)

    def sample(self, o, d, jitter: Optional[torch.Tensor], training: bool, keep_feat: bool = False,
               begun: Optional[dict] = None, device_counts=False) -> Packed:
        c = self.cfg
        st = begun if begun is not None else self.sample_begin(o, d, jitter, training, device_counts=device_counts)
        learn = device_counts and st["mode"] == 0 and self.device_counts_ok()
        dc_now = learn and device_counts is True and "n0" not in st
        if st.get("dc") is not None and not dc_now:
            st = self.sample_begin(o, d, jitter, training)
        args, cache, counts, offsets, mode = st["args"], st["cache"], st["counts"], st["offsets"], st["mode"]
        if dc_now:
            caps = st["dc"]["caps"] if st.get("dc") is not None else self.counts.capacities(o.shape[0])
            if caps is not None:
                return self._sample_device_counts(o, d, st, caps, keep_feat)
        n0 = st["n0"] if "n0" in st else _host_int(st["total"])
        ri, ts, te = ops.ray_march_write(*args, offsets, n0, counts=counts, cache=cache)
        if mode == 1 or n0 == 0:
            if learn:
                self.counts.learn(o.shape[0], n0, n0)
            return Packed(ri, ts, te, offsets, counts, n0, n0)
        keep_feat = keep_feat and self._reuse_prepass_feat and c.mlp_kernels == "x"
        sigma = self._density_stream(o, d, (ri, ts, te), n0, keep_feat)
        feat0 = None
        if keep_feat:
            sigma, feat0 = sigma
        keep, kept = ops.visibility(offsets, counts, sigma, ts, te, c.early_stop_eps, c.alpha_thre)
        new_offsets, total2 = ops.exclusive_scan(kept)
        n1 = _host_int(total2)
        ri2, ts2, te2 = ops.compact_samples(offsets, counts, new_offsets, keep, ts, te, n1)
        feat1 = None
        if feat0 is not None and n1 > 0:
            feat1 = feat0 if n1 == n0 else ops.compact_features(offsets, counts, new_offsets, keep, feat0, n1)
        if learn:
            self.counts.learn(o.shape[0], n0, n1)
        return Packed(ri2, ts2, te2, new_offsets, kept, n1, n0, feat1)

    def _mlp_params(self):
        m = self.field.mlp
        return m.to(torch.bfloat16).to(torch.float32) if self.cfg.mlp_bf16 else m

    def _density_stream(self, o, d, samples, n, return_feat: bool = False, n_dev=None):
        feat = ops.hashgrid_fwd(self.field.grid, self.field.table, scene=self.scene, rays=(o, d),
                                samples=samples, n=n, layout=1, n_dev=n_dev)
        if self.cfg.mlp_kernels == "x":
            _, sigma, _, _ = ops.mlp_fwd_x(self.field.mlp, self.field.C, self._xmode(), feat, self.scene, rays=(o, d),
                                           samples=samples, n=n, density_only=True, act=self._act_code, n_dev=n_dev)
            return (sigma, feat) if return_feat else sigma
        _, sigma, _ = ops.mlp_fwd(self._mlp_params(), self.field.C, feat, self.scene, rays=(o, d),
                                  samples=samples, n=n, density_only=True, bf16=self.cfg.mlp_bf16, act=self._act_code)
        return sigma

    def _binned_workspace(self, n: int, device) -> torch.Tensor:
        need = ops.hashgrid_bwd_binned_workspace_bytes(n)
        ws = self._bin_ws
        if self._capture is not None:
            if ws is None or ws.numel() < need:
                raise RuntimeError("binned-scatter workspace too small for the step being captured")
            return ws
        if ws is not None and ws.numel() >= need:
            self._bin_ws_small = self._bin_ws_small + 1 if ws.numel() > 4 * need else 0
            if self._bin_ws_small < 32:
                return ws
        shrink = ws is not None and ws.numel() >= need
        del ws
        self._bin_ws = None
        self._bin_ws_small = 0
        if shrink:
            torch.cuda.empty_cache()
        self._bin_ws = torch.empty(need + need // 4, device=device, dtype=torch.uint8)
        return self._bin_ws

    def _save_acts(self) -> bool:
        c = self.cfg
        return (c.mlp_kernels != "x") if c.save_activations is None else bool(c.save_activations)

    def _xmode(self) -> int:
        return 1 if self.cfg.mlp_bf16 else 3 if self.cfg.mlp_precision == "high" else 6

    def _field_forward(self, o, d, pk, save):
        f = self.field
        samples = (pk.ray_indices, pk.t_starts, pk.t_ends)
        chunks = min(self.cfg.fwd_chunks, pk.n >> 20) if pk.n >= (1 << 23) else 1
        if self.cfg.mlp_kernels == "x" and chunks > 1 and pk.feat is None and pk.n_dev is None:
            return self._field_forward_chunked(o, d, pk, save, chunks)
        feat = pk.feat if pk.feat is not None else \
            ops.hashgrid_fwd(f.grid, f.table, scene=self.scene, rays=(o, d), samples=samples, n=pk.n, layout=1, n_dev=pk.n_dev)
        if self.cfg.mlp_kernels == "x":
            rgb, sigma, base, acts = ops.mlp_fwd_x(f.mlp, f.C, self._xmode(), feat, self.scene, rays=(o, d), samples=samples,
                                                   n=pk.n, save=save, save_acts=self._save_acts(), act=self._act_code, n_dev=pk.n_dev)
            return rgb, sigma, dict(feat=feat, base=base, acts=acts, xmode=self._xmode() if save else None)
        mp = self._mlp_params()
        if save and self._save_acts():
            rgb, sigma, base, acts = ops.mlp_fwd_save(mp, f.C, feat, self.scene, rays=(o, d), samples=samples, n=pk.n,
                                                      bf16=self.cfg.mlp_bf16, act=self._act_code)
            return rgb, sigma, dict(feat=feat, base=base, mlp_params=mp, acts=acts)
        rgb, sigma, base = ops.mlp_fwd(mp, f.C, feat, self.scene, rays=(o, d), samples=samples, n=pk.n,
                                       save_base=save, bf16=self.cfg.mlp_bf16, act=self._act_code)
        return rgb, sigma, dict(feat=feat, base=base, mlp_params=mp)

    def _field_forward_chunked(self, o, d, pk, save, K):
        f, n = self.field, pk.n
        dev = o.device
        lib_acts = ops.mlp_act_save_floats(32)
        nblk = ops.n_blocks32(n)
        per = -(-nblk // K)
        feat = torch.empty(nblk * ops.FRAG_FLOATS_PER_BLOCK, device=dev)
        sigma = torch.empty(n, device=dev)
        rgb = torch.empty(n, f.C, device=dev)
        base = torch.empty(nblk * ops.BASE_FLOATS_PER_BLOCK, device=dev) if save else None
        acts = torch.empty(nblk * lib_acts, device=dev) if (save and self._save_acts()) else None
        if self._fwd_streams is None:
            self._fwd_streams = (torch.cuda.Stream(dev), torch.cuda.Stream(dev))
        main = torch.cuda.current_stream()
        s_enc, s_mlp = self._fwd_streams
        s_enc.wait_stream(main)
        s_mlp.wait_stream(main)
        for k in range(K):
            b0, b1 = k * per, min(nblk, (k + 1) * per)
            if b0 >= b1:
                break
            lo, hi = b0 * 32, min(n, b1 * 32)
            smp = (pk.ray_indices[lo:hi], pk.t_starts[lo:hi], pk.t_ends[lo:hi])
            fk = feat[b0 * ops.FRAG_FLOATS_PER_BLOCK: b1 * ops.FRAG_FLOATS_PER_BLOCK]
            with torch.cuda.stream(s_enc):
                ops.hashgrid_fwd(f.grid, f.table, scene=self.scene, rays=(o, d), samples=smp, n=hi - lo, layout=1, out=fk)
                ev = torch.cuda.Event()
                ev.record(s_enc)
            with torch.cuda.stream(s_mlp):
                s_mlp.wait_event(ev)
                out = (rgb[lo:hi], sigma[lo:hi],
                       base[b0 * ops.BASE_FLOATS_PER_BLOCK: b1 * ops.BASE_FLOATS_PER_BLOCK] if save else None,
                       acts[b0 * lib_acts: b1 * lib_acts] if acts is not None else None)
                ops.mlp_fwd_x(f.mlp, f.C, self._xmode(), fk, self.scene, rays=(o, d), samples=smp, n=hi - lo, save=save,
                              out=out, share_cu=True, act=self._act_code)
        main.wait_stream(s_enc)
        main.wait_stream(s_mlp)
        return rgb, sigma, dict(feat=feat, base=base, acts=acts, xmode=self._xmode() if save else None)

    def dp_early_slice(self) -> Optional[Tuple[int, int]]:
        if self.grad_sync is None or not self.cfg.dp_overlap or not self.cfg.binned_scatter or not self.dp_early_enabled:
            return None
        f = self.field
        return 2 * int(f.grid.offset[self.cfg.dp_split_level]), f.n_table

    def dp_early(self):
        a, b = self.dp_early_slice()
        self.grad_sync.early(self.field.grad_all, a, b)

    def _field_backward_chunked(self, ctx, d_rgb, d_sig, K: int):
        f, pk = self.field, ctx["pk"]
        n, dev = pk.n, d_rgb.device
        nblk = ops.n_blocks32(n)
        per = -(-nblk // K)
        FR, BA = ops.FRAG_FLOATS_PER_BLOCK, ops.BASE_FLOATS_PER_BLOCK
        dfeat = torch.empty(nblk * FR, device=dev)
        d_base = torch.empty(nblk * BA, device=dev)
        ws = self._binned_workspace(n, dev)
        rays, samples = (ctx["o"], ctx["d"]), (pk.ray_indices, pk.t_starts, pk.t_ends)
        if self._bwd_stream is None:
            self._bwd_stream = torch.cuda.Stream(dev)
        main, side = torch.cuda.current_stream(), self._bwd_stream
        ops.hashgrid_bwd_binned_begin(f.grid, ws, scene=self.scene, rays=rays, samples=samples, n=n)
        side.wait_stream(main)
        acts_per = ops.mlp_act_save_floats(32)
        for k in range(K):
            b0, b1 = k * per, min(nblk, (k + 1) * per)
            if b0 >= b1:
                break
            lo, hi = b0 * 32, min(n, b1 * 32)
            acts = ctx["acts"][b0 * acts_per: b1 * acts_per] if ctx.get("acts") is not None else None
            ops.mlp_bwd_x(f.mlp, f.C, ctx["xmode"], ctx["feat"][b0 * FR: b1 * FR], ctx["base"][b0 * BA: b1 * BA], acts,
                          self.scene, rays=rays, samples=tuple(t[lo:hi] for t in samples), n=hi - lo,
                          rgb=ctx["rgb"][lo:hi], d_rgb=d_rgb[lo:hi], d_sigma=d_sig[lo:hi], grad_mlp_params=f.g_mlp,
                          workspace=self._ws, dfeat=dfeat[b0 * FR: b1 * FR], d_base=d_base[b0 * BA: b1 * BA],
                          act=self._act_code, grid_cus=0 if k == 0 else self.cfg.bwd_mlp_cus)
            ev = torch.cuda.Event()
            ev.record(main)
            with torch.cuda.stream(side):
                side.wait_event(ev)
                ops.hashgrid_bwd_binned_scatter(f.grid, f.g_table, dfeat, ws, scene=self.scene, rays=rays, samples=samples,
                                                n=n, first=lo, m=hi - lo)
        main.wait_stream(side)
        ops.hashgrid_bwd_binned_finish(f.grid, f.g_table, ws, n=n)

    def _field_backward(self, ctx, d_rgb, d_sig, final: bool = False):
        f, pk = self.field, ctx["pk"]
        K = min(self.cfg.bwd_chunks, pk.n >> 21) if pk.n >= (1 << 23) else 1
        if (K > 1 and ctx.get("xmode") is not None and self.cfg.binned_scatter and pk.n_dev is None and
                not (final and self.dp_early_slice() is not None)):
            return self._field_backward_chunked(ctx, d_rgb, d_sig, K)
        samples = (pk.ray_indices, pk.t_starts, pk.t_ends)
        mp = ctx.get("mlp_params")
        if ctx.get("xmode") is not None:
            cus = torch.cuda.get_device_properties(d_rgb.device).multi_processor_count - self.bwd_side_cus if self.bwd_side_cus else 0
            dfeat = ops.mlp_bwd_x(f.mlp, f.C, ctx["xmode"], ctx["feat"], ctx["base"], ctx["acts"], self.scene,
                                  rays=(ctx["o"], ctx["d"]), samples=samples, n=pk.n, rgb=ctx["rgb"], d_rgb=d_rgb,
                                  d_sigma=d_sig, grad_mlp_params=f.g_mlp, workspace=self._ws, act=self._act_code, n_dev=pk.n_dev,
                                  grid_cus=max(cus, 0))
        elif ctx.get("acts") is not None:
            dfeat = ops.mlp_bwd_saved(mp, f.C, ctx["feat"], ctx["base"], ctx["acts"], self.scene, rays=(ctx["o"], ctx["d"]),
                                      samples=samples, n=pk.n, rgb=ctx["rgb"], d_rgb=d_rgb, d_sigma=d_sig,
                                      grad_mlp_params=f.g_mlp, workspace=self._ws, bf16=self.cfg.mlp_bf16, act=self._act_code)
        else:
            dfeat = ops.mlp_bwd(f.mlp if mp is None else mp, f.C, ctx["feat"], ctx["base"], self.scene,
                                rays=(ctx["o"], ctx["d"]), samples=samples, n=pk.n, rgb=ctx["rgb"], d_rgb=d_rgb,
                                d_sigma=d_sig, grad_mlp_params=f.g_mlp, workspace=self._ws,
                                bf16=self.cfg.mlp_bf16 and mp is not None, act=self._act_code)
        if self.cfg.binned_scatter:
            self._binned_workspace(pk.n, dfeat.device)
            kw = dict(scene=self.scene, rays=(ctx["o"], ctx["d"]), samples=samples, n=pk.n, layout=1, n_dev=pk.n_dev)
            if final and self.dp_early_slice() is not None:
                lo_mask = (1 << self.cfg.dp_split_level) - 1
                ops.hashgrid_bwd_binned(f.grid, f.g_table, dfeat, self._bin_ws, level_mask=0xFFFF & ~lo_mask, **kw)
                self.dp_early()
                ops.hashgrid_bwd_binned(f.grid, f.g_table, dfeat, self._bin_ws, level_mask=lo_mask, **kw)
            else:
                ops.hashgrid_bwd_binned(f.grid, f.g_table, dfeat, self._bin_ws, **kw)
        else:
            ops.hashgrid_bwd(f.grid, f.g_table, dfeat, scene=self.scene, rays=(ctx["o"], ctx["d"]), samples=samples,
                             n=pk.n, layout=1)

    def forward(self, o, d, jitter=None, bkgd: Optional[torch.Tensor] = None, training: bool = True,
                save: bool = True, begun: Optional[dict] = None, device_counts: bool = False):
        f = self.field
        pk = self.sample(o, d, jitter, training, keep_feat=True, begun=begun, device_counts=device_counts)
        n_rays = o.shape[0]
        if pk.n == 0:
            colors = torch.zeros(n_rays, f.C, device=o.device)
            if bkgd is not None:
                colors = colors + bkgd
            zero = torch.zeros(n_rays, device=o.device)
            return colors, zero, zero.clone(), dict(pk=pk, empty=True, bkgd=bkgd)
        rgb, sigma, fctx = self._field_forward(o, d, pk, save)
        colors, opac, depth, w, T = ops.composite_fwd(pk.offsets, pk.counts, pk.t_starts, pk.t_ends, sigma, rgb,
                                                      f.C, bkgd, save=save)
        ctx = dict(pk=pk, o=o, d=d, rgb=rgb, sigma=sigma, w=w, T=T, opac=opac, bkgd=bkgd, empty=False, **fctx)
        return colors, opac, depth, ctx

    def backward(self, ctx, g_colors, g_opac=None, g_depth=None, final: bool = False, per_ray_bkgd: bool = False):
        f = self.field
        if ctx["empty"]:
            if final and self.dp_early_slice() is not None:
                self.dp_early()
            if ctx.get("bkgd") is None:
                return None
            return g_colors if per_ray_bkgd else g_colors.sum(0)
        pk = ctx["pk"]
        d_sig, d_rgb, d_bk = ops.composite_bwd(pk.offsets, pk.counts, pk.t_starts, pk.t_ends, ctx["sigma"],
                                               ctx["rgb"], f.C, ctx["bkgd"], ctx["w"], ctx["T"], ctx["opac"],
                                               g_colors, g_opac, g_depth, want_bkgd=ctx["bkgd"] is not None)
        self._field_backward(ctx, d_rgb, d_sig, final=final)
        if per_ray_bkgd:
            return d_bk
        return ops.column_sum(d_bk) if d_bk is not None else None

    def query_density(self, x_world: torch.Tensor) -> torch.Tensor:
        f = self.field
        n = x_world.shape[0]
        xu = contract_points(x_world, self.cfg.aabb, self.cfg.contraction_type)
        feat = ops.hashgrid_fwd(f.grid, f.table, x_unit=xu, n=n, layout=1)
        if self.cfg.mlp_kernels == "x":
            return ops.mlp_fwd_x(f.mlp, f.C, self._xmode(), feat, self.scene, x_world=x_world, n=n, density_only=True, act=self._act_code)[1]
        _, sigma, _ = ops.mlp_fwd(self._mlp_params(), f.C, feat, self.scene, x_world=x_world, n=n, density_only=True,
                                  bf16=self.cfg.mlp_bf16, act=self._act_code)
        return sigma

    def _density_gradient_stream(self, o, d, samples, n):
        f = self.field
        dev = f.flat.device
        if self._normal_scratch is None:
            self._normal_scratch = torch.empty(f.n_mlp, device=dev, dtype=torch.float32)
        self._normal_scratch.zero_()
        feat = ops.hashgrid_fwd(f.grid, f.table, scene=self.scene, rays=(o, d), samples=samples, n=n, layout=1)
        mp = f.mlp
        _, sigma, base = ops.mlp_fwd(mp, f.C, feat, self.scene, rays=(o, d), samples=samples, n=n, density_only=True,
                                     save_base=True, act=self._act_code)
        zero_rgb = torch.zeros(n, f.C, device=dev, dtype=torch.float32)
        dfeat = ops.mlp_bwd(mp, f.C, feat, base, self.scene, rays=(o, d), samples=samples, n=n, rgb=zero_rgb, d_rgb=zero_rgb,
# ... 514 lines not shown
```

### robust_e_nerf_amd/ops.py

```python
from __future__ import annotations

import ctypes
import math
from typing import Optional, Sequence, Tuple

import torch

from . import _lib
from ._lib import GridDesc, SceneDesc, check

AABB, UN_BOUNDED_TANH, UN_BOUNDED_SPHERE = 0, 1, 2
FRAG_FLOATS_PER_BLOCK = 16 * 64
BASE_FLOATS_PER_BLOCK = 8 * 64

_DT = {torch.float32: 4, torch.float64: 8, torch.int32: 4, torch.int64: 8, torch.uint8: 1, torch.bool: 1}


KNOBS = {"hgb_no_pairs": 0, "hgb_halve_regions": 1, "march_sequential": 2, "hg_variant": 3, "vfield_plain": 4, "hgb_subregion": 5}


class knob:

    def __init__(self, name: str, value: int):
        self.k, self.v = KNOBS[name], int(value)
# ... 68 lines not shown
        scale = np.float32(np.exp2(np.float32(lvl) * log2_pls).astype(np.float32) * np.float32(base_resolution)
                           - np.float32(1.0))
        res = int(np.ceil(scale)) + 1
        dense = res ** 3
        size = (min(dense, 2 ** 31 - 1) + 7) // 8 * 8
        if otype == "HashGrid":
            size = min(size, 1 << log2_hashmap_size)
        elif otype == "TiledGrid":
            size = min(size, base_resolution ** 3)
        if offset + size >= 1 << 32:
            raise NotImplementedError("grid with more than 2^32 entries")
        g.scale[lvl] = float(scale)
        g.res[lvl] = res
        g.size[lvl] = size
        g.offset[lvl] = offset
        g.hashed[lvl] = 1 if (otype == "HashGrid" and dense > size) else 0
        offset += size
    return g, offset * 2


def make_scene_desc(aabb: Sequence[float], contraction_type: int) -> SceneDesc:
    s = SceneDesc()
    for k in range(6):
        s.aabb[k] = float(aabb[k])
    s.contraction_type = int(contraction_type)
    return s


def mlp_param_count(radiance_dim: int = 1) -> int:
    return 9360 + 65 * radiance_dim


MLP_SLICES = {
}


def mlp_slices(C: int = 1):
    return {
        "base.w0": (0, (64, 32)), "base.b0": (2048, (64,)), "base.wo": (2112, (16, 64)), "base.bo": (3136, (16,)),
        "head.w0": (3152, (64, 31)), "head.b0": (5136, (64,)), "head.w1": (5200, (64, 64)), "head.b1": (9296, (64,)),
        "head.wo": (9360, (C, 64)), "head.bo": (9360 + 64 * C, (C,)),
    }


def weight_norm_layers(layers):
    import ctypes
    flat = [int(v) for layer in layers for v in layer]
    return (ctypes.c_int32 * len(flat))(*flat), len(layers)


def weight_norm_fwd(raw, g, table, eff):
    import ctypes
    arr, n_layers = table
    check(_lib.load().ren_weight_norm_fwd(_ptr(raw), _ptr(g), ctypes.cast(arr, ctypes.c_void_p), n_layers, raw.numel(),
                                          _ptr(eff), _stream()), "ren_weight_norm_fwd")
    return eff


def weight_norm_bwd(raw, g, d_eff, table, d_raw, d_g, zero_d_eff: bool = False):
    import ctypes
    arr, n_layers = table
    check(_lib.load().ren_weight_norm_bwd(_ptr(raw), _ptr(g), _ptr(d_eff), ctypes.cast(arr, ctypes.c_void_p), n_layers,
                                          raw.numel(), _ptr(d_raw), _ptr(d_g), int(zero_d_eff), _stream()),
          "ren_weight_norm_bwd")


def n_blocks32(n: int) -> int:
    return (n + 31) // 32


def trajectory(ts: torch.Tensor, tab_ts, tab_pos, tab_quat):
    B = ts.shape[0]
    pos = torch.empty(B, 3, device=ts.device, dtype=torch.float32)
    rot = torch.empty(B, 3, 3, device=ts.device, dtype=torch.float32)
    check(_lib.load().ren_trajectory_fwd(_ptr(ts, torch.float64), B, _ptr(tab_ts, torch.int64),
                                         _ptr(tab_pos, torch.float32), _ptr(tab_quat, torch.float32),
                                         tab_ts.shape[0], _ptr(pos), _ptr(rot), _stream()), "ren_trajectory_fwd")
    return pos, rot


def raygen(Kinv, px, pos, rot):
    B = px.shape[0]
    o = torch.empty(B, 3, device=px.device, dtype=torch.float32)
    d = torch.empty(B, 3, device=px.device, dtype=torch.float32)
    check(_lib.load().ren_raygen_fwd(_ptr(Kinv, torch.float32), _ptr(px, torch.float32), _ptr(pos, torch.float32),
                                     _ptr(rot, torch.float32), B, _ptr(o), _ptr(d), _stream()), "ren_raygen_fwd")
    return o, d


def pose_rays(ts, px, Kinv, tab_ts, tab_pos, tab_quat):
    R = ts.shape[0]
    o = torch.empty(R, 3, device=ts.device, dtype=torch.float32)
    d = torch.empty(R, 3, device=ts.device, dtype=torch.float32)
    check(_lib.load().ren_pose_rays_fwd(_ptr(ts, torch.float64), R, _ptr(px, torch.float32), px.shape[0], _ptr(Kinv, torch.float32),
                                        _ptr(tab_ts, torch.int64), _ptr(tab_pos, torch.float32), _ptr(tab_quat, torch.float32),
                                        tab_ts.shape[0], _ptr(o), _ptr(d), _stream()), "ren_pose_rays_fwd")
    return o, d


def ray_aabb_intersect(o, d, aabb: Sequence[float], near: Optional[float] = None, far: Optional[float] = None):
    n = o.shape[0]
    tmin = torch.empty(n, device=o.device, dtype=torch.float32)
    tmax = torch.empty(n, device=o.device, dtype=torch.float32)
    ab = (ctypes.c_float * 6)(*[float(v) for v in aabb])
    check(_lib.load().ren_ray_aabb_intersect(_ptr(o, torch.float32), _ptr(d, torch.float32), n, ab,
                                             _f(NAN if near is None else near), _f(NAN if far is None else far),
                                             _ptr(tmin), _ptr(tmax), _stream()), "ren_ray_aabb_intersect")
    return tmin, tmax


def uniform(n: int, seed: int, offset: int = 0, device="cuda:0", out=None):
    if out is None:
        out = torch.empty(n, device=device, dtype=torch.float32)
    check(_lib.load().ren_uniform(int(seed) & (2 ** 64 - 1), int(offset) & (2 ** 64 - 1), n, _ptr(out), _stream()), "ren_uniform")
    return out


def exclusive_scan(counts: torch.Tensor):
    n = counts.shape[0]
    offsets = torch.empty(n, device=counts.device, dtype=torch.int64)
    total = torch.empty(1, device=counts.device, dtype=torch.int64)
    scratch = torch.empty(1024, device=counts.device, dtype=torch.int64) if n > 65536 else None
    check(_lib.load().ren_exclusive_scan(_ptr(counts, torch.int32), n, _ptr(offsets), _ptr(total), _ptr(scratch),
                                         _stream()), "ren_exclusive_scan")
    return offsets, total


MARCH_VERIFIED_DIV = 0x100


def march_div_check(roi, device) -> bool:
    ext = [float(roi[3 + k]) - float(roi[k]) for k in range(3)]
    if not all(2.0 ** -59 < e < 2.0 ** 59 for e in ext) or not all(2.0 ** -59 < abs(float(roi[k])) < 2.0 ** 59 for k in range(3)):
        return False
    roi_c = (ctypes.c_float * 6)(*[float(v) for v in roi])
    out = torch.zeros(1, dtype=torch.int64, device=device)
    check(_lib.load().ren_march_div_check(roi_c, _ptr(out, torch.int64), _stream()), "ren_march_div_check")
    return int(out.item()) == 0


def ray_march_count(o, d, t_min, t_max, jitter, roi, res, binary, ct, step, cone, mode, n_uniform, cache=None):
    n = o.shape[0]
    counts = torch.empty(n, device=o.device, dtype=torch.int32)
    roi_c = (ctypes.c_float * 6)(*[float(v) for v in roi])
    res_c = (ctypes.c_int32 * 3)(*[int(v) for v in res])
    check(_lib.load().ren_ray_march(_ptr(o), _ptr(d), _ptr(t_min), _ptr(t_max), _ptr(jitter), n, roi_c, res_c,
                                    _ptr(binary, (torch.uint8, torch.bool)), ct, _f(step), _f(cone), mode, n_uniform,
                                    None, _ptr(counts), None, None, None, _ptr(cache, torch.float32),
                                    0 if cache is None else cache.shape[1], _stream()), "ren_ray_march(count)")
    return counts


def ray_march_write(o, d, t_min, t_max, jitter, roi, res, binary, ct, step, cone, mode, n_uniform,
                    offsets, n_total: int, out=None, counts=None, cache=None):
    n = o.shape[0]
    if out is None:
        ri = torch.empty(n_total, device=o.device, dtype=torch.int32)
        ts = torch.empty(n_total, device=o.device, dtype=torch.float32)
        te = torch.empty(n_total, device=o.device, dtype=torch.float32)
    else:
        ri, ts, te = out
    if n_total == 0:
        return ri, ts, te
    roi_c = (ctypes.c_float * 6)(*[float(v) for v in roi])
    res_c = (ctypes.c_int32 * 3)(*[int(v) for v in res])
    check(_lib.load().ren_ray_march(_ptr(o), _ptr(d), _ptr(t_min), _ptr(t_max), _ptr(jitter), n, roi_c, res_c,
                                    _ptr(binary, (torch.uint8, torch.bool)), ct, _f(step), _f(cone), mode, n_uniform,
                                    _ptr(offsets, torch.int64), _ptr(counts, torch.int32), _ptr(ri), _ptr(ts), _ptr(te),
                                    _ptr(cache, torch.float32) if counts is not None else None,
                                    0 if (cache is None or counts is None) else cache.shape[1], _stream()),
          "ren_ray_march(write)")
    return ri, ts, te


def count_guard(counts, total, capacity: int, n_out, stats=None, counts_also=None):
    check(_lib.load().ren_count_guard(_ptr(counts, torch.int32), _ptr(counts_also, torch.int32), counts.shape[0],
                                      _ptr(total, torch.int64), int(capacity), _ptr(n_out, torch.int64), _ptr(stats, torch.int64),
                                      _stream()), "ren_count_guard")


def scan_guard(counts, capacity: int, n_out, stats=None, counts_also=None):
    n = counts.shape[0]
    offsets = torch.empty(n, device=counts.device, dtype=torch.int64)
    total = torch.empty(1, device=counts.device, dtype=torch.int64)
    scratch = torch.empty(1024, device=counts.device, dtype=torch.int64) if n > 65536 else None
    check(_lib.load().ren_scan_guard(_ptr(counts, torch.int32), _ptr(counts_also, torch.int32), n, _ptr(offsets), _ptr(total),
                                     int(capacity), _ptr(n_out, torch.int64), _ptr(stats, torch.int64), _ptr(scratch), _stream()),
          "ren_scan_guard")
    return offsets, total


def frag_zero_tail(feat, capacity: int, n_dev):
    check(_lib.load().ren_frag_zero_tail(_ptr(feat, torch.float32), int(capacity), _ptr(n_dev, torch.int64), _stream()),
          "ren_frag_zero_tail")


def visibility(offsets, counts, sigmas, ts, te, eps: float, alpha_thre: float):
    n_rays = counts.shape[0]
    keep = torch.empty(ts.shape[0], device=ts.device, dtype=torch.uint8)
    kept = torch.empty(n_rays, device=ts.device, dtype=torch.int32)
    check(_lib.load().ren_visibility(_ptr(offsets, torch.int64), _ptr(counts, torch.int32), n_rays,
                                     _ptr(sigmas, torch.float32), _ptr(ts), _ptr(te), _f(eps), _f(alpha_thre),
                                     _ptr(keep), _ptr(kept), _stream()), "ren_visibility")
    return keep, kept


def compact_samples(offsets, counts, new_offsets, keep, ts, te, n_new: int):
    n_rays = counts.shape[0]
    ri2 = torch.empty(n_new, device=ts.device, dtype=torch.int32)
    ts2 = torch.empty(n_new, device=ts.device, dtype=torch.float32)
    te2 = torch.empty(n_new, device=ts.device, dtype=torch.float32)
    if n_new == 0:
        return ri2, ts2, te2
    check(_lib.load().ren_compact_samples(_ptr(offsets), _ptr(counts), _ptr(new_offsets), n_rays, _ptr(keep),
                                          _ptr(ts), _ptr(te), _ptr(ri2), _ptr(ts2), _ptr(te2), _stream()),
          "ren_compact_samples")
    return ri2, ts2, te2


def compact_features(offsets, counts, new_offsets, keep, feat, n_new: int, n_dev=None):
    out = torch.empty(n_blocks32(n_new) * FRAG_FLOATS_PER_BLOCK, device=feat.device, dtype=torch.float32)
    if n_new == 0:
        return out
    if n_dev is None:
        out[-FRAG_FLOATS_PER_BLOCK:].zero_()
    check(_lib.load().ren_compact_features(_ptr(offsets, torch.int64), _ptr(counts, torch.int32), _ptr(new_offsets, torch.int64),
                                           counts.shape[0], _ptr(keep), _ptr(feat, torch.float32), _ptr(out), _stream()),
          "ren_compact_features")
    if n_dev is not None:
        frag_zero_tail(out, n_new, n_dev)
    return out


def pack_info(ray_indices: torch.Tensor, n_rays: int):
    n = ray_indices.shape[0]
    offsets = torch.empty(n_rays, device=ray_indices.device, dtype=torch.int64)
    counts = torch.empty(n_rays, device=ray_indices.device, dtype=torch.int32)
    check(_lib.load().ren_pack_info(_ptr(ray_indices, torch.int32), n, n_rays, _ptr(offsets), _ptr(counts),
                                    _stream()), "ren_pack_info")
    return offsets, counts


def hashgrid_fwd(grid: GridDesc, table, *, x_unit=None, scene: Optional[SceneDesc] = None, rays=None,
                 samples=None, n: int, layout: int, out=None, n_dev=None):
    L = grid.n_levels
    dev = table.device
    if out is None:
        out = (torch.empty(n, 2 * L, device=dev, dtype=torch.float32) if layout == 0
               else torch.empty(n_blocks32(n) * FRAG_FLOATS_PER_BLOCK, device=dev, dtype=torch.float32))
    o, d = rays if rays is not None else (None, None)
    ri, ts, te = samples if samples is not None else (None, None, None)
    check(_lib.load().ren_hashgrid_fwd(ctypes.byref(grid), _ptr(table, torch.float32), _ptr(x_unit),
                                       ctypes.byref(scene) if scene is not None else None,
                                       _ptr(o), _ptr(d), _ptr(ri), _ptr(ts), _ptr(te), n, layout, _ptr(out), _ptr(n_dev, torch.int64),
                                       _stream()), "ren_hashgrid_fwd")
    return out


def hashgrid_bwd(grid: GridDesc, grad_table, dfeat, *, x_unit=None, scene=None, rays=None, samples=None,
                 n: int, layout: int):
    o, d = rays if rays is not None else (None, None)
    ri, ts, te = samples if samples is not None else (None, None, None)
    check(_lib.load().ren_hashgrid_bwd(ctypes.byref(grid), _ptr(grad_table, torch.float32), _ptr(x_unit),
                                       ctypes.byref(scene) if scene is not None else None,
                                       _ptr(o), _ptr(d), _ptr(ri), _ptr(ts), _ptr(te), n, layout,
                                       _ptr(dfeat, torch.float32), _stream()), "ren_hashgrid_bwd")


def hashgrid_bwd_input(grid: GridDesc, table, dfeat, *, x_unit=None, scene=None, rays=None, samples=None,
                       n: int, layout: int, out=None):
    if out is None:
        out = torch.empty(n, 3, device=table.device, dtype=torch.float32)
    if n == 0:
        return out
    o, d = rays if rays is not None else (None, None)
    ri, ts, te = samples if samples is not None else (None, None, None)
    check(_lib.load().ren_hashgrid_bwd_input(ctypes.byref(grid), _ptr(table, torch.float32), _ptr(x_unit),
                                             ctypes.byref(scene) if scene is not None else None,
                                             _ptr(o), _ptr(d), _ptr(ri), _ptr(ts), _ptr(te), n, layout,
                                             _ptr(dfeat, torch.float32), _ptr(out, torch.float32), _stream()),
          "ren_hashgrid_bwd_input")
    return out


def hashgrid_bwd_binned_workspace_bytes(n: int) -> int:
    return int(_lib.load().ren_hashgrid_bwd_binned_workspace_bytes(n))


def hashgrid_bwd_binned(grid: GridDesc, grad_table, dfeat, workspace, *, x_unit=None, scene=None, rays=None,
                        samples=None, n: int, layout: int, level_mask: Optional[int] = None, tangent=None, n_dev=None):
    if workspace.numel() * workspace.element_size() < hashgrid_bwd_binned_workspace_bytes(n):
        raise ValueError("hashgrid_bwd_binned: workspace too small")
    o, d = rays if rays is not None else (None, None)
    ri, ts, te = samples if samples is not None else (None, None, None)
    if level_mask is not None or tangent is not None:
        do, dd, dfd = tangent if tangent is not None else (None, None, None)
        check(_lib.load().ren_hashgrid_bwd_binned_levels(
            ctypes.byref(grid), _ptr(grad_table, torch.float32), _ptr(x_unit), ctypes.byref(scene) if scene is not None else None,
            _ptr(o), _ptr(d), _ptr(ri), _ptr(ts), _ptr(te), n, layout, _ptr(dfeat, torch.float32), _ptr(do), _ptr(dd), _ptr(dfd),
            0xFFFFFFFF if level_mask is None else int(level_mask), _ptr(workspace), _ptr(n_dev, torch.int64), _stream()),
              "ren_hashgrid_bwd_binned_levels")
        return
    check(_lib.load().ren_hashgrid_bwd_binned(ctypes.byref(grid), _ptr(grad_table, torch.float32), _ptr(x_unit),
                                              ctypes.byref(scene) if scene is not None else None,
                                              _ptr(o), _ptr(d), _ptr(ri), _ptr(ts), _ptr(te), n, layout,
                                              _ptr(dfeat, torch.float32), _ptr(workspace), _ptr(n_dev, torch.int64), _stream()),
          "ren_hashgrid_bwd_binned")


BINNED_MAX_LEVEL_ENTRIES = 1 << 19


def binned_supported(grid: GridDesc) -> bool:
    return max(int(grid.size[l]) for l in range(grid.n_levels)) <= BINNED_MAX_LEVEL_ENTRIES


def hashgrid_bwd_auto(grid: GridDesc, grad_table, dfeat, *, x_unit=None, scene=None, rays=None, samples=None, n: int,
                      layout: int):
    if binned_supported(grid):
        ws = torch.empty(hashgrid_bwd_binned_workspace_bytes(n), device=dfeat.device, dtype=torch.uint8)
        hashgrid_bwd_binned(grid, grad_table, dfeat, ws, x_unit=x_unit, scene=scene, rays=rays, samples=samples, n=n,
                            layout=layout)
    else:
        hashgrid_bwd(grid, grad_table, dfeat, x_unit=x_unit, scene=scene, rays=rays, samples=samples, n=n, layout=layout)


def hashgrid_bwd_binned_begin(grid: GridDesc, workspace, *, scene, rays, samples, n: int, layout: int = 1):
    if workspace.numel() * workspace.element_size() < hashgrid_bwd_binned_workspace_bytes(n):
        raise ValueError("hashgrid_bwd_binned: workspace too small")
    (o, d), (ri, ts, te) = rays, samples
    check(_lib.load().ren_hashgrid_bwd_binned_begin(ctypes.byref(grid), None, ctypes.byref(scene), _ptr(o), _ptr(d), _ptr(ri),
                                                    _ptr(ts), _ptr(te), n, layout, _ptr(workspace), _stream()),
          "ren_hashgrid_bwd_binned_begin")


def hashgrid_bwd_binned_scatter(grid: GridDesc, grad_table, dfeat, workspace, *, scene, rays, samples, n: int, first: int,
                                m: int, layout: int = 1):
    (o, d), (ri, ts, te) = rays, samples
    check(_lib.load().ren_hashgrid_bwd_binned_scatter(ctypes.byref(grid), _ptr(grad_table, torch.float32), None, ctypes.byref(scene),
                                                      _ptr(o), _ptr(d), _ptr(ri), _ptr(ts), _ptr(te), n, layout,
                                                      _ptr(dfeat, torch.float32), first, m, _ptr(workspace), _stream()),
          "ren_hashgrid_bwd_binned_scatter")


def hashgrid_bwd_binned_finish(grid: GridDesc, grad_table, workspace, *, n: int, layout: int = 1):
    check(_lib.load().ren_hashgrid_bwd_binned_finish(ctypes.byref(grid), _ptr(grad_table, torch.float32), n, layout,
                                                     _ptr(workspace), _stream()), "ren_hashgrid_bwd_binned_finish")


def mlp_fwd(mlp_params, C: int, feat, scene: SceneDesc, *, x_world=None, dirs=None, rays=None, samples=None,
            n: int, density_only: bool = False, save_base: bool = False, out=None, bf16: bool = False, act: int = 0):
    dev = feat.device
    o, d = rays if rays is not None else (None, None)
    ri, ts, te = samples if samples is not None else (None, None, None)
    if out is None:
        sigma = torch.empty(n, device=dev, dtype=torch.float32)
        rgb = None if density_only else torch.empty(n, C, device=dev, dtype=torch.float32)
        base = torch.empty(n_blocks32(n) * BASE_FLOATS_PER_BLOCK, device=dev, dtype=torch.float32) if save_base else None
    else:
        rgb, sigma, base = out
    fn = _lib.load().ren_mlp_fwd_bf16 if bf16 else _lib.load().ren_mlp_fwd
    check(fn(_ptr(mlp_params, torch.float32), C, int(act), _ptr(feat, torch.float32), ctypes.byref(scene),
             _ptr(x_world), _ptr(dirs), _ptr(o), _ptr(d), _ptr(ri), _ptr(ts), _ptr(te), n,
             1 if density_only else 0, _ptr(rgb), _ptr(sigma), _ptr(base), _stream()),
# ... 659 lines not shown
```

Baseline: 6.151 million rays/s.

## Precompute contracted unit positions in ray march and fuse dense hashgrid levels

The ray-march kernels now also write contracted unit-cube sample positions (x_unit). Compaction carries these positions forward, so the hashgrid forward and density passes read them directly instead of recomputing positions from rays for every level. Separately, the hashgrid forward kernel merges the leading non-hashed (dense) levels into one block that loops over them, which means fewer grid rows and a single position load for those levels. In exchange the march writes 12 extra bytes per sample and holds an extra buffer, and fast fp contraction can shift rounding slightly.

```diff
diff --git a/include/ren_amd.h b/include/ren_amd.h
--- a/include/ren_amd.h
+++ b/include/ren_amd.h
@@ -60,6 +60,14 @@
                   const int64_t *offsets, int32_t *counts,
                   int32_t *ray_indices, float *t_starts, float *t_ends, float *interval_cache,
                   int32_t cache_cap, void *stream);
+int ren_ray_march_unit(const float *rays_o, const float *rays_d, const float *t_min,
+                       const float *t_max, const float *jitter, int64_t n_rays,
+                       const float *roi_host, const int32_t *res_host, const uint8_t *binary,
+                       int32_t contraction_type, float step_size, float cone_angle,
+                       int32_t mode, int32_t n_uniform,
+                       const int64_t *offsets, int32_t *counts,
+                       int32_t *ray_indices, float *t_starts, float *t_ends, float *interval_cache,
+                       int32_t cache_cap, const ren_scene_desc *scene, float *x_unit, void *stream);
 
 int ren_march_div_check(const float *roi, int64_t *mismatches, void *stream);
 int ren_uniform(uint64_t seed, uint64_t offset, int64_t n, float *out, void *stream);
@@ -80,6 +88,10 @@
                         int64_t n_rays, const uint8_t *keep, const float *t_starts,
                         const float *t_ends, int32_t *out_ray_indices, float *out_t_starts,
                         float *out_t_ends, void *stream);
+int ren_compact_samples_unit(const int64_t *offsets, const int32_t *counts, const int64_t *new_offsets,
+                             int64_t n_rays, const uint8_t *keep, const float *t_starts,
+                             const float *t_ends, const float *x_unit, int32_t *out_ray_indices, float *out_t_starts,
+                             float *out_t_ends, float *out_x_unit, void *stream);
 int ren_compact_features(const int64_t *offsets, const int32_t *counts, const int64_t *new_offsets, int64_t n_rays,
                          const uint8_t *keep, const float *feat_in, float *feat_out, void *stream);
 int ren_pack_info(const int32_t *ray_indices, int64_t n, int64_t n_rays, int64_t *offsets,
@@ -89,6 +101,9 @@
                      const ren_scene_desc *scene, const float *rays_o, const float *rays_d,
                      const int32_t *ray_indices, const float *t_starts, const float *t_ends,
                      int64_t n, int32_t layout, float *feat, const int64_t *n_dev, void *stream);
+int ren_unit_positions(const ren_scene_desc *scene, const float *rays_o, const float *rays_d,
+                       const int32_t *ray_indices, const float *t_starts, const float *t_ends, int64_t n,
+                       float *x_unit, const int64_t *n_dev, void *stream);
 int ren_hashgrid_bwd(const ren_grid_desc *grid, float *grad_table, const float *x_unit,
                      const ren_scene_desc *scene, const float *rays_o, const float *rays_d,
                      const int32_t *ray_indices, const float *t_starts, const float *t_ends,
diff --git a/robust_e_nerf_amd/_lib.py b/robust_e_nerf_amd/_lib.py
--- a/robust_e_nerf_amd/_lib.py
+++ b/robust_e_nerf_amd/_lib.py
@@ -38,6 +38,10 @@
     "ren_march_div_check": (c_int, [POINTER(c_float), P, P]),
     "ren_ray_march": (c_int, [P, P, P, P, P, c_int64, POINTER(c_float), POINTER(c_int32), P, c_int32,
                               c_float, c_float, c_int32, c_int32, P, P, P, P, P, P, c_int32, P]),
+    "ren_ray_march_unit": (c_int, [P, P, P, P, P, c_int64, POINTER(c_float), POINTER(c_int32), P, c_int32,
+                                   c_float, c_float, c_int32, c_int32, P, P, P, P, P, P, c_int32, POINTER(SceneDesc), P, P]),
+    "ren_compact_samples_unit": (c_int, [P, P, P, c_int64, P, P, P, P, P, P, P, P, P]),
+    "ren_unit_positions": (c_int, [POINTER(SceneDesc), P, P, P, P, P, c_int64, P, P, P]),
     "ren_compact_features": (c_int, [P, P, P, c_int64, P, P, P, P]),
     "ren_uniform": (c_int, [ctypes.c_uint64, ctypes.c_uint64, c_int64, P, P]),
     "ren_exclusive_scan": (c_int, [P, c_int64, P, P, P, P]),
diff --git a/robust_e_nerf_amd/csrc/ren_common.h b/robust_e_nerf_amd/csrc/ren_common.h
--- a/robust_e_nerf_amd/csrc/ren_common.h
+++ b/robust_e_nerf_amd/csrc/ren_common.h
@@ -62,6 +62,9 @@
 
 __device__ __forceinline__ void ren_contract(const ren_scene_dev &sc, float x, float y, float z,
                                              float &ux, float &uy, float &uz) {
+#ifdef REN_FUSED_POSITIONS
+#pragma clang fp contract(fast)
+#endif
     ux = (x - sc.lo[0]) / (sc.hi[0] - sc.lo[0]);
     uy = (y - sc.lo[1]) / (sc.hi[1] - sc.lo[1]);
     uz = (z - sc.lo[2]) / (sc.hi[2] - sc.lo[2]);
@@ -94,6 +97,25 @@
     z = o[2] + d[2] * tm;
 }
 
+__device__ __forceinline__ void ren_sample_pos_at(const float *o, const float *d, float t0, float t1,
+                                                  float &x, float &y, float &z) {
+#ifdef REN_FUSED_POSITIONS
+#pragma clang fp contract(fast)
+#endif
+    float tm = (t0 + t1) * 0.5f;
+    x = o[0] + d[0] * tm;
+    y = o[1] + d[1] * tm;
+    z = o[2] + d[2] * tm;
+}
+
+__device__ __forceinline__ void ren_store_unit_pos(const ren_scene_dev &sc, const float *o, const float *d, float t0, float t1,
+                                                   float *__restrict__ x_unit, int64_t at) {
+    float x, y, z, ux, uy, uz;
+    ren_sample_pos_at(o, d, t0, t1, x, y, z);
+    ren_contract(sc, x, y, z, ux, uy, uz);
+    x_unit[3 * at] = ux; x_unit[3 * at + 1] = uy; x_unit[3 * at + 2] = uz;
+}
+
 __device__ __forceinline__ int64_t ren_eff_n(int64_t n, const int64_t *__restrict__ n_dev) {
     if (!n_dev) return n;
     const int64_t m = *n_dev;
diff --git a/robust_e_nerf_amd/csrc/ren_hashgrid.hip b/robust_e_nerf_amd/csrc/ren_hashgrid.hip
--- a/robust_e_nerf_amd/csrc/ren_hashgrid.hip
+++ b/robust_e_nerf_amd/csrc/ren_hashgrid.hip
@@ -21,18 +21,21 @@
     const float *__restrict__ rays_o, const float *__restrict__ rays_d,
     const int32_t *__restrict__ ray_indices, const float *__restrict__ t_starts,
     const float *__restrict__ t_ends, int64_t n, int64_t n_pad, float *__restrict__ feat, int xcd_affine,
-    const int64_t *__restrict__ n_dev) {
+    const int64_t *__restrict__ n_dev, int n_fuse) {
     int lvl; int64_t chunk;
     if (!block_to_work(xcd_affine, g.n_levels, (n_pad + 255) / 256, lvl, chunk)) return;
+    int lvl_end = lvl + 1;
+    if (n_fuse > 1) {
+        if (lvl == 0) lvl_end = n_fuse; else { lvl += n_fuse - 1; lvl_end = lvl + 1; }
+    }
     const int64_t i = chunk * blockDim.x + threadIdx.x;
     if (n_dev) {
         n = ren_eff_n(n, n_dev);
         if (LAYOUT == 1) { const int64_t p = ((n + 31) >> 5) << 5; n_pad = p < n_pad ? p : n_pad; } else n_pad = n;
     }
     if (i >= n_pad) return;
-    float f0 = 0.f, f1 = 0.f;
+    float ux = 0.f, uy = 0.f, uz = 0.f;
     if (i < n) {
-        float ux, uy, uz;
         if (FROM_RAYS) {
             float x, y, z; int ray;
             ren_sample_pos(rays_o, rays_d, ray_indices, t_starts, t_ends, i, x, y, z, ray);
@@ -40,31 +43,51 @@
         } else {
             ux = x_unit[3 * i]; uy = x_unit[3 * i + 1]; uz = x_unit[3 * i + 2];
         }
-        const LevelPos p = level_pos(ux, uy, uz, g.scale[lvl]);
-        const uint32_t res = g.res[lvl], size = g.size[lvl];
-        const bool hashed = g.hashed[lvl] != 0;
-        const float2 *tab = table + g.offset[lvl];
-        float2 v[8];
-        uint32_t idx[8];
-        corner_indices8(p.c[0], p.c[1], p.c[2], res, size, hashed, idx);
-        gather_corners8(tab, idx, v);
+    }
+#pragma unroll 1
+    for (; lvl < lvl_end; ++lvl) {
+        float f0 = 0.f, f1 = 0.f;
+        if (i < n) {
+            const LevelPos p = level_pos(ux, uy, uz, g.scale[lvl]);
+            const uint32_t res = g.res[lvl], size = g.size[lvl];
+            const bool hashed = g.hashed[lvl] != 0;
+            const float2 *tab = table + g.offset[lvl];
+            float2 v[8];
+            uint32_t idx[8];
+            corner_indices8(p.c[0], p.c[1], p.c[2], res, size, hashed, idx);
+            gather_corners8(tab, idx, v);
 #pragma unroll
-        for (int c = 0; c < 8; ++c) {
-            const float wx = (c & 1) ? p.w[0] : 1.f - p.w[0];
-            const float wy = (c & 2) ? p.w[1] : 1.f - p.w[1];
-            const float wz = (c & 4) ? p.w[2] : 1.f - p.w[2];
-            const float w = wx * wy * wz;
-            f0 += w * v[c].x;
-            f1 += w * v[c].y;
-        }
-    }
-    if (LAYOUT == 0) {
-        if (i < n) reinterpret_cast<float2 *>(feat)[i * g.n_levels + lvl] = make_float2(f0, f1);
-    } else {
-        const int64_t b = ((i >> 5) * REN_MAX_LEVELS + lvl) * 64 + (i & 31);
-        __builtin_nontemporal_store(f0, feat + b);
-        __builtin_nontemporal_store(f1, feat + b + 32);
-    }
+            for (int c = 0; c < 8; ++c) {
+                const float wx = (c & 1) ? p.w[0] : 1.f - p.w[0];
+                const float wy = (c & 2) ? p.w[1] : 1.f - p.w[1];
+                const float wz = (c & 4) ? p.w[2] : 1.f - p.w[2];
+                const float w = wx * wy * wz;
+                f0 += w * v[c].x;
+                f1 += w * v[c].y;
+            }
+        }
+        if (LAYOUT == 0) {
+            if (i < n) reinterpret_cast<float2 *>(feat)[i * g.n_levels + lvl] = make_float2(f0, f1);
+        } else {
+            const int64_t b = ((i >> 5) * REN_MAX_LEVELS + lvl) * 64 + (i & 31);
+            __builtin_nontemporal_store(f0, feat + b);
+            __builtin_nontemporal_store(f1, feat + b + 32);
+        }
+    }
+}
+
+__global__ __launch_bounds__(256) void unit_positions_kernel(ren_scene_dev sc, const float *__restrict__ rays_o,
+                                                             const float *__restrict__ rays_d,
+                                                             const int32_t *__restrict__ ray_indices,
+                                                             const float *__restrict__ t_starts,
+                                                             const float *__restrict__ t_ends, int64_t n,
+                                                             const int64_t *__restrict__ n_dev, float *__restrict__ x_unit) {
+    const int64_t i = (int64_t)blockIdx.x * blockDim.x + threadIdx.x;
+    if (i >= ren_eff_n(n, n_dev)) return;
+    float x, y, z, ux, uy, uz; int ray;
+    ren_sample_pos(rays_o, rays_d, ray_indices, t_starts, t_ends, i, x, y, z, ray);
+    ren_contract(sc, x, y, z, ux, uy, uz);
+    x_unit[3 * i] = ux; x_unit[3 * i + 1] = uy; x_unit[3 * i + 2] = uz;
 }
 
 template <int LAYOUT, bool FROM_RAYS, bool PAIR>
@@ -144,16 +167,31 @@
     const int variant = hg_variant();
     const int affine = variant & 5;
     const int64_t n_chunks = (n_pad + 255) / 256;
+    int n_fuse = 0;
+    if (!affine && !(variant & 8))
+        while (n_fuse < g.n_levels && !g.hashed[n_fuse]) ++n_fuse;
+    if (n_fuse < 2) n_fuse = 0;
     dim3 grd = (affine & 4) ? dim3((unsigned)(g.n_levels * n_chunks))
-             : affine ? dim3((unsigned)(8 * ((g.n_levels + 7) / 8) * n_chunks)) : dim3((unsigned)n_chunks, g.n_levels);
+             : affine ? dim3((unsigned)(8 * ((g.n_levels + 7) / 8) * n_chunks))
+             : dim3((unsigned)n_chunks, n_fuse ? g.n_levels - n_fuse + 1 : g.n_levels);
     dim3 blk(256);
     const float2 *tab = reinterpret_cast<const float2 *>(table);
 #define LAUNCH(L, R)                                                                                     \
     hipLaunchKernelGGL((hashgrid_fwd_kernel<L, R>), grd, blk, 0, (hipStream_t)stream, g, tab, x_unit, sc, \
-                       rays_o, rays_d, ray_indices, t_starts, t_ends, n, n_pad, feat, affine, n_dev)
+                       rays_o, rays_d, ray_indices, t_starts, t_ends, n, n_pad, feat, affine, n_dev, n_fuse)
     if (layout == 0) { if (from_rays) LAUNCH(0, true); else LAUNCH(0, false); }
     else             { if (from_rays) LAUNCH(1, true); else LAUNCH(1, false); }
 #undef LAUNCH
+    REN_CHECK_LAUNCH();
+}
+
+extern "C" int ren_unit_positions(const ren_scene_desc *scene, const float *rays_o, const float *rays_d,
+                                  const int32_t *ray_indices, const float *t_starts, const float *t_ends, int64_t n,
+                                  float *x_unit, const int64_t *n_dev, void *stream) {
+    if (!scene || !rays_o || !rays_d || !ray_indices || !t_starts || !t_ends || !x_unit || n < 0) return REN_ERR_BAD_ARG;
+    if (n == 0) return REN_OK;
+    hipLaunchKernelGGL(unit_positions_kernel, dim3(ren_blocks(n, 256)), dim3(256), 0, (hipStream_t)stream, ren_make_scene(scene),
+                       rays_o, rays_d, ray_indices, t_starts, t_ends, n, n_dev, x_unit);
     REN_CHECK_LAUNCH();
 }
 
diff --git a/robust_e_nerf_amd/csrc/ren_sampling.hip b/robust_e_nerf_amd/csrc/ren_sampling.hip
--- a/robust_e_nerf_amd/csrc/ren_sampling.hip
+++ b/robust_e_nerf_amd/csrc/ren_sampling.hip
@@ -1,3 +1,4 @@
+#define REN_FUSED_POSITIONS
 #include "ren_common.h"
 #include <cstdlib>
 
@@ -125,7 +126,8 @@
                                  const uint8_t *__restrict__ binary,
                                  const int64_t *__restrict__ offsets, int32_t *__restrict__ counts,
                                  int32_t *__restrict__ ray_indices, float *__restrict__ t_starts,
-                                 float *__restrict__ t_ends, float2 *__restrict__ cache, int cache_cap) {
+                                 float *__restrict__ t_ends, float2 *__restrict__ cache, int cache_cap,
+                                 ren_scene_dev sc, float *__restrict__ x_unit) {
     int64_t i = (int64_t)blockIdx.x * blockDim.x + threadIdx.x;
     if (i >= n_rays) return;
     if (WRITE && cache && counts[i] <= cache_cap) return;
@@ -146,6 +148,7 @@
                     t_starts[base + j] = t0;
                     t_ends[base + j] = t0 + delta;
                     ray_indices[base + j] = (int32_t)i;
+                    if (x_unit) ren_store_unit_pos(sc, ro, rd, t0, t0 + delta, x_unit, base + j);
                 }
             }
             j = a.n_uniform;
@@ -168,6 +171,7 @@
                 t_starts[base + j] = t0;
                 t_ends[base + j] = t1;
                 ray_indices[base + j] = (int32_t)i;
+                if (x_unit) ren_store_unit_pos(sc, ro, rd, t0, t1, x_unit, base + j);
             } else if (cache && j < cache_cap) {
                 cache[i * cache_cap + j] = make_float2(t0, t1);
             }
@@ -196,7 +200,7 @@
     const float *__restrict__ t_max, const float *__restrict__ jitter, int64_t n_rays, MarchArgs a,
     const uint8_t *__restrict__ binary, const int64_t *__restrict__ offsets, int32_t *__restrict__ counts,
     int32_t *__restrict__ ray_indices, float *__restrict__ t_starts, float *__restrict__ t_ends,
-    float2 *__restrict__ cache, int cache_cap) {
+    float2 *__restrict__ cache, int cache_cap, ren_scene_dev sc, float *__restrict__ x_unit) {
     const int64_t i = ((int64_t)blockIdx.x * blockDim.x + threadIdx.x) / SPEC;
     const int l = threadIdx.x % SPEC, lane = threadIdx.x & 63, g0 = lane - l;
     bool done = i >= n_rays;
@@ -285,6 +289,7 @@
                 t_starts[base + at] = a0;
                 t_ends[base + at] = a1;
                 ray_indices[base + at] = (int32_t)i;
+                if (x_unit) ren_store_unit_pos(sc, ro, rd, a0, a1, x_unit, base + at);
             } else if (cache && at < cache_cap) {
                 cache[i * cache_cap + at] = make_float2(a0, a1);
             }
@@ -313,7 +318,9 @@
                                                            const int64_t *__restrict__ offsets,
                                                            const int32_t *__restrict__ counts,
                                                            int32_t *__restrict__ ray_indices, float *__restrict__ t_starts,
-                                                           float *__restrict__ t_ends) {
+                                                           float *__restrict__ t_ends, const float *__restrict__ o,
+                                                           const float *__restrict__ d, ren_scene_dev sc,
+                                                           float *__restrict__ x_unit) {
     const int64_t g = (int64_t)blockIdx.x * blockDim.x + threadIdx.x;
     const int64_t i = g >> 3;
     if (i >= n_rays) return;
@@ -321,11 +328,17 @@
     if (c > cache_cap) return;
     const int64_t base = offsets[i];
     const float2 *src = cache + i * cache_cap;
+    float ro[3] = {0.f, 0.f, 0.f}, rd[3] = {0.f, 0.f, 0.f};
+    if (x_unit) {
+#pragma unroll
+        for (int k = 0; k < 3; ++k) { ro[k] = o[3 * i + k]; rd[k] = d[3 * i + k]; }
+    }
     for (int j = (int)(g & 7); j < c; j += 8) {
         const float2 v = src[j];
         t_starts[base + j] = v.x;
         t_ends[base + j] = v.y;
         ray_indices[base + j] = (int32_t)i;
+        if (x_unit) ren_store_unit_pos(sc, ro, rd, v.x, v.y, x_unit, base + j);
     }
 }
 
@@ -333,7 +346,9 @@
                                                             const float *__restrict__ jitter, int64_t n_rays, int n_uniform,
                                                             const int64_t *__restrict__ offsets,
                                                             int32_t *__restrict__ ray_indices, float *__restrict__ t_starts,
-                                                            float *__restrict__ t_ends) {
+                                                            float *__restrict__ t_ends, const float *__restrict__ o,
+                                                            const float *__restrict__ d, ren_scene_dev sc,
+                                                            float *__restrict__ x_unit) {
     const int64_t g = (int64_t)blockIdx.x * blockDim.x + threadIdx.x;
     const int64_t i = g / n_uniform;
     const int j = (int)(g - i * n_uniform);
@@ -347,6 +362,10 @@
     t_starts[at] = t0;
     t_ends[at] = t0 + delta;
     ray_indices[at] = (int32_t)i;
+    if (x_unit) {
+        const float ro[3] = {o[3 * i], o[3 * i + 1], o[3 * i + 2]}, rd[3] = {d[3 * i], d[3 * i + 1], d[3 * i + 2]};
+        ren_store_unit_pos(sc, ro, rd, t0, t0 + delta, x_unit, at);
+    }
 }
 
 constexpr int SCAN_TILE = 1024;
@@ -456,7 +475,8 @@
                                const int64_t *__restrict__ new_offsets, int64_t n_rays,
                                const uint8_t *__restrict__ keep, const float *__restrict__ t_starts,
                                const float *__restrict__ t_ends, int32_t *__restrict__ out_ri,
-                               float *__restrict__ out_ts, float *__restrict__ out_te) {
+                               float *__restrict__ out_ts, float *__restrict__ out_te,
+                               const float *__restrict__ x_unit, float *__restrict__ out_xu) {
     const int64_t i = ((int64_t)blockIdx.x * blockDim.x + threadIdx.x) >> 6;
     const int lane = threadIdx.x & 63;
     if (i >= n_rays) return;
@@ -473,6 +493,10 @@
             out_ri[at] = (int32_t)i;
             out_ts[at] = t_starts[j];
             out_te[at] = t_ends[j];
+            if (out_xu) {
+#pragma unroll
+                for (int k = 0; k < 3; ++k) out_xu[3 * at + k] = x_unit[3 * j + k];
+            }
         }
         w += __popcll(m);
     }
@@ -577,14 +601,17 @@
     REN_CHECK_LAUNCH();
 }
 
-extern "C" int ren_ray_march(const float *rays_o, const float *rays_d, const float *t_min,
-                             const float *t_max, const float *jitter, int64_t n_rays,
-                             const float *roi, const int32_t *res, const uint8_t *binary,
-                             int32_t contraction_type, float step_size, float cone_angle,
-                             int32_t mode, int32_t n_uniform, const int64_t *offsets, int32_t *counts,
-                             int32_t *ray_indices, float *t_starts, float *t_ends, float *interval_cache,
-                             int32_t cache_cap, void *stream) {
+static int ray_march_impl(const float *rays_o, const float *rays_d, const float *t_min,
+                          const float *t_max, const float *jitter, int64_t n_rays,
+                          const float *roi, const int32_t *res, const uint8_t *binary,
+                          int32_t contraction_type, float step_size, float cone_angle,
+                          int32_t mode, int32_t n_uniform, const int64_t *offsets, int32_t *counts,
+                          int32_t *ray_indices, float *t_starts, float *t_ends, float *interval_cache,
+                          int32_t cache_cap, const ren_scene_desc *scene, float *x_unit, void *stream) {
     if (!rays_o || !rays_d || !t_min || !t_max || n_rays < 0) return REN_ERR_BAD_ARG;
+    if (x_unit && (!scene || !t_starts)) return REN_ERR_BAD_ARG;
+    ren_scene_dev sc = {};
+    if (scene) sc = ren_make_scene(scene);
     const bool verified_div = (mode & REN_MARCH_VERIFIED_DIV) != 0;
     mode &= ~REN_MARCH_VERIFIED_DIV;
     if (mode != 0 && mode != 1) return REN_ERR_BAD_ARG;
@@ -617,42 +644,68 @@
         if (width == 16)                                                                                                   \
             hipLaunchKernelGGL((ray_march_spec_kernel<WRITE, 16>), sgrid, dim3(256), 0, (hipStream_t)stream, rays_o, rays_d, \
                                t_min, t_max, jitter, n_rays, a, binary, offsets, counts, ray_indices, t_starts, t_ends,    \
-                               cache, cache_cap);                                                                          \
+                               cache, cache_cap, sc, x_unit);                                                              \
         else if (width == 8)                                                                                               \
             hipLaunchKernelGGL((ray_march_spec_kernel<WRITE, 8>), sgrid, dim3(256), 0, (hipStream_t)stream, rays_o, rays_d, \
                                t_min, t_max, jitter, n_rays, a, binary, offsets, counts, ray_indices, t_starts, t_ends,    \
-                               cache, cache_cap);                                                                          \
+                               cache, cache_cap, sc, x_unit);                                                              \
         else if (width == 4)                                                                                               \
             hipLaunchKernelGGL((ray_march_spec_kernel<WRITE, 4>), sgrid, dim3(256), 0, (hipStream_t)stream, rays_o, rays_d, \
                                t_min, t_max, jitter, n_rays, a, binary, offsets, counts, ray_indices, t_starts, t_ends,    \
-                               cache, cache_cap);                                                                          \
+                               cache, cache_cap, sc, x_unit);                                                              \
         else                                                                                                               \
             hipLaunchKernelGGL((ray_march_spec_kernel<WRITE, 2>), sgrid, dim3(256), 0, (hipStream_t)stream, rays_o, rays_d, \
                                t_min, t_max, jitter, n_rays, a, binary, offsets, counts, ray_indices, t_starts, t_ends,    \
-                               cache, cache_cap);                                                                          \
+                               cache, cache_cap, sc, x_unit);                                                              \
     } while (0)
     if (write && mode == 1)
         hipLaunchKernelGGL(uniform_write_kernel, dim3(ren_blocks(n_rays * n_uniform, 256)), dim3(256), 0,
                            (hipStream_t)stream, t_min, t_max, jitter, n_rays, n_uniform, offsets, ray_indices,
-                           t_starts, t_ends);
+                           t_starts, t_ends, rays_o, rays_d, sc, x_unit);
     else if (write) {
         if (cache)
             hipLaunchKernelGGL(cached_write_kernel, dim3(ren_blocks(n_rays * 8, 256)), dim3(256), 0, (hipStream_t)stream,
-                               cache, cache_cap, n_rays, offsets, counts, ray_indices, t_starts, t_ends);
+                               cache, cache_cap, n_rays, offsets, counts, ray_indices, t_starts, t_ends, rays_o, rays_d, sc,
+                               x_unit);
         if (width)
             REN_MARCH_SPEC(true);
         else
             hipLaunchKernelGGL(ray_march_kernel<true>, grid, block, 0, (hipStream_t)stream, rays_o, rays_d,
                                t_min, t_max, jitter, n_rays, a, binary, offsets, counts, ray_indices,
-                               t_starts, t_ends, cache, cache_cap);
+                               t_starts, t_ends, cache, cache_cap, sc, x_unit);
     } else if (width)
         REN_MARCH_SPEC(false);
     else
         hipLaunchKernelGGL(ray_march_kernel<false>, grid, block, 0, (hipStream_t)stream, rays_o, rays_d,
                            t_min, t_max, jitter, n_rays, a, binary, offsets, counts, ray_indices,
-                           t_starts, t_ends, cache, cache_cap);
+                           t_starts, t_ends, cache, cache_cap, sc, x_unit);
 #undef REN_MARCH_SPEC
     REN_CHECK_LAUNCH();
+}
+
+extern "C" int ren_ray_march(const float *rays_o, const float *rays_d, const float *t_min,
+                             const float *t_max, const float *jitter, int64_t n_rays,
+                             const float *roi, const int32_t *res, const uint8_t *binary,
+                             int32_t contraction_type, float step_size, float cone_angle,
+                             int32_t mode, int32_t n_uniform, const int64_t *offsets, int32_t *counts,
+                             int32_t *ray_indices, float *t_starts, float *t_ends, float *interval_cache,
+                             int32_t cache_cap, void *stream) {
+    return ray_march_impl(rays_o, rays_d, t_min, t_max, jitter, n_rays, roi, res, binary, contraction_type, step_size,
+                          cone_angle, mode, n_uniform, offsets, counts, ray_indices, t_starts, t_ends, interval_cache,
+                          cache_cap, nullptr, nullptr, stream);
+}
+
+extern "C" int ren_ray_march_unit(const float *rays_o, const float *rays_d, const float *t_min,
+                                  const float *t_max, const float *jitter, int64_t n_rays,
+                                  const float *roi, const int32_t *res, const uint8_t *binary,
+                                  int32_t contraction_type, float step_size, float cone_angle,
+                                  int32_t mode, int32_t n_uniform, const int64_t *offsets, int32_t *counts,
+                                  int32_t *ray_indices, float *t_starts, float *t_ends, float *interval_cache,
+                                  int32_t cache_cap, const ren_scene_desc *scene, float *x_unit, void *stream) {
+    if (!scene || !x_unit || !t_starts) return REN_ERR_BAD_ARG;
+    return ray_march_impl(rays_o, rays_d, t_min, t_max, jitter, n_rays, roi, res, binary, contraction_type, step_size,
+                          cone_angle, mode, n_uniform, offsets, counts, ray_indices, t_starts, t_ends, interval_cache,
+                          cache_cap, scene, x_unit, stream);
 }
 
 __global__ __launch_bounds__(256) void philox_uniform_kernel(uint64_t seed, uint64_t offset, int64_t n, float *__restrict__ out) {
@@ -838,19 +891,38 @@
     REN_CHECK_LAUNCH();
 }
 
-extern "C" int ren_compact_samples(const int64_t *offsets, const int32_t *counts,
-                                   const int64_t *new_offsets, int64_t n_rays, const uint8_t *keep,
-                                   const float *t_starts, const float *t_ends,
-                                   int32_t *out_ray_indices, float *out_t_starts, float *out_t_ends,
-                                   void *stream) {
+static int compact_samples_impl(const int64_t *offsets, const int32_t *counts,
+                                const int64_t *new_offsets, int64_t n_rays, const uint8_t *keep,
+                                const float *t_starts, const float *t_ends,
+                                int32_t *out_ray_indices, float *out_t_starts, float *out_t_ends,
+                                const float *x_unit, float *out_x_unit, void *stream) {
     if (!offsets || !counts || !new_offsets || !keep || !t_starts || !t_ends || !out_ray_indices ||
         !out_t_starts || !out_t_ends || n_rays < 0)
         return REN_ERR_BAD_ARG;
     if (n_rays == 0) return REN_OK;
     hipLaunchKernelGGL(compact_kernel, dim3(ren_blocks(n_rays * 64, 256)), dim3(256), 0, (hipStream_t)stream,
                        offsets, counts, new_offsets, n_rays, keep, t_starts, t_ends, out_ray_indices,
-                       out_t_starts, out_t_ends);
-    REN_CHECK_LAUNCH();
+                       out_t_starts, out_t_ends, x_unit, out_x_unit);
+    REN_CHECK_LAUNCH();
+}
+
+extern "C" int ren_compact_samples(const int64_t *offsets, const int32_t *counts,
+                                   const int64_t *new_offsets, int64_t n_rays, const uint8_t *keep,
+                                   const float *t_starts, const float *t_ends,
+                                   int32_t *out_ray_indices, float *out_t_starts, float *out_t_ends,
+                                   void *stream) {
+    return compact_samples_impl(offsets, counts, new_offsets, n_rays, keep, t_starts, t_ends, out_ray_indices, out_t_starts,
+                                out_t_ends, nullptr, nullptr, stream);
+}
+
+extern "C" int ren_compact_samples_unit(const int64_t *offsets, const int32_t *counts,
+                                        const int64_t *new_offsets, int64_t n_rays, const uint8_t *keep,
+                                        const float *t_starts, const float *t_ends, const float *x_unit,
+                                        int32_t *out_ray_indices, float *out_t_starts, float *out_t_ends,
+                                        float *out_x_unit, void *stream) {
+    if (!x_unit || !out_x_unit) return REN_ERR_BAD_ARG;
+    return compact_samples_impl(offsets, counts, new_offsets, n_rays, keep, t_starts, t_ends, out_ray_indices, out_t_starts,
+                                out_t_ends, x_unit, out_x_unit, stream);
 }
 
 extern "C" int ren_compact_features(const int64_t *offsets, const int32_t *counts, const int64_t *new_offsets,
diff --git a/robust_e_nerf_amd/engine.py b/robust_e_nerf_amd/engine.py
--- a/robust_e_nerf_amd/engine.py
+++ b/robust_e_nerf_amd/engine.py
@@ -158,6 +158,7 @@
     feat: Optional[torch.Tensor] = None
     n_dev: Optional[torch.Tensor] = None
     log: Optional["CountLog"] = None
+    x_unit: Optional[torch.Tensor] = None
 
 
 def pack_batch(batch: Dict[str, torch.Tensor]) -> Dict[str, torch.Tensor]:
@@ -294,6 +295,9 @@
         return (c.device_counts is not False and c.sampler == "occgrid" and type(self) is Renderer and c.mlp_kernels == "x" and
                 c.binned_scatter and self.field.flat.is_cuda)
 
+    def _unit_scene(self):
+        return self.scene if (type(self) is Renderer and getattr(self.field, "grid", None) is not None) else None
+
     def _sample_device_counts(self, o, d, st, caps, keep_feat: bool) -> Packed:
         c = self.cfg
         args, cache, counts, offsets = st["args"], st["cache"], st["counts"], st["offsets"]
@@ -304,18 +308,20 @@
             ops.count_guard(counts, st["total"], caps[0], nd[0:1], stats[0:2])
         cap0, cap1 = caps
         n0_dev, n1_dev = nd[0:1], nd[1:2]
-        ri, ts, te = ops.ray_march_write(*args, offsets, cap0, counts=counts, cache=cache)
+        ri, ts, te, *xu = ops.ray_march_write(*args, offsets, cap0, counts=counts, cache=cache, unit_scene=self._unit_scene())
+        xu = xu[0] if xu else None
         keep_feat = keep_feat and self._reuse_prepass_feat
-        sigma = self._density_stream(o, d, (ri, ts, te), cap0, keep_feat, n_dev=n0_dev)
+        sigma = self._density_stream(o, d, (ri, ts, te), cap0, keep_feat, n_dev=n0_dev, x_unit=xu)
         feat0 = None
         if keep_feat:
             sigma, feat0 = sigma
         keep, kept = ops.visibility(offsets, counts, sigma, ts, te, c.early_stop_eps, c.alpha_thre)
         new_offsets, total2 = ops.scan_guard(kept, cap1, n1_dev, stats[2:4], counts_also=counts)
-        ri2, ts2, te2 = ops.compact_samples(offsets, counts, new_offsets, keep, ts, te, cap1)
+        ri2, ts2, te2, *xu2 = ops.compact_samples(offsets, counts, new_offsets, keep, ts, te, cap1,
+                                                  x_unit=xu if feat0 is None else None)
         feat1 = ops.compact_features(offsets, counts, new_offsets, keep, feat0, cap1, n_dev=n1_dev) if feat0 is not None else None
         log = self.counts.log(o.shape[0], caps, stats, self._capture)
-        return Packed(ri2, ts2, te2, new_offsets, kept, cap1, cap0, feat1, n_dev=n1_dev, log=log)
+        return Packed(ri2, ts2, te2, new_offsets, kept, cap1, cap0, feat1, n_dev=n1_dev, log=log, x_unit=xu2[0] if xu2 else None)
 
     def sample(self, o, d, jitter: Optional[torch.Tensor], training: bool, keep_feat: bool = False,
                begun: Optional[dict] = None, device_counts=False) -> Packed:
@@ -331,34 +337,41 @@
             if caps is not None:
                 return self._sample_device_counts(o, d, st, caps, keep_feat)
         n0 = st["n0"] if "n0" in st else _host_int(st["total"])
-        ri, ts, te = ops.ray_march_write(*args, offsets, n0, counts=counts, cache=cache)
+        ri, ts, te, *xu = ops.ray_march_write(*args, offsets, n0, counts=counts, cache=cache, unit_scene=self._unit_scene())
+        xu = xu[0] if xu else None
         if mode == 1 or n0 == 0:
             if learn:
                 self.counts.learn(o.shape[0], n0, n0)
-            return Packed(ri, ts, te, offsets, counts, n0, n0)
+            return Packed(ri, ts, te, offsets, counts, n0, n0, x_unit=xu)
         keep_feat = keep_feat and self._reuse_prepass_feat and c.mlp_kernels == "x"
-        sigma = self._density_stream(o, d, (ri, ts, te), n0, keep_feat)
+        sigma = self._density_stream(o, d, (ri, ts, te), n0, keep_feat, **({} if xu is None else dict(x_unit=xu)))
         feat0 = None
         if keep_feat:
             sigma, feat0 = sigma
         keep, kept = ops.visibility(offsets, counts, sigma, ts, te, c.early_stop_eps, c.alpha_thre)
         new_offsets, total2 = ops.exclusive_scan(kept)
         n1 = _host_int(total2)
-        ri2, ts2, te2 = ops.compact_samples(offsets, counts, new_offsets, keep, ts, te, n1)
+        ri2, ts2, te2, *xu2 = ops.compact_samples(offsets, counts, new_offsets, keep, ts, te, n1,
+                                                  x_unit=xu if feat0 is None else None)
         feat1 = None
         if feat0 is not None and n1 > 0:
             feat1 = feat0 if n1 == n0 else ops.compact_features(offsets, counts, new_offsets, keep, feat0, n1)
         if learn:
             self.counts.learn(o.shape[0], n0, n1)
-        return Packed(ri2, ts2, te2, new_offsets, kept, n1, n0, feat1)
+        return Packed(ri2, ts2, te2, new_offsets, kept, n1, n0, feat1, x_unit=xu2[0] if xu2 else None)
 
     def _mlp_params(self):
         m = self.field.mlp
         return m.to(torch.bfloat16).to(torch.float32) if self.cfg.mlp_bf16 else m
 
-    def _density_stream(self, o, d, samples, n, return_feat: bool = False, n_dev=None):
-        feat = ops.hashgrid_fwd(self.field.grid, self.field.table, scene=self.scene, rays=(o, d),
-                                samples=samples, n=n, layout=1, n_dev=n_dev)
+    def _hash_features(self, o, d, samples, n, x_unit=None, n_dev=None, out=None):
+        f = self.field
+        if x_unit is not None:
+            return ops.hashgrid_fwd(f.grid, f.table, x_unit=x_unit, n=n, layout=1, n_dev=n_dev, out=out)
+        return ops.hashgrid_fwd(f.grid, f.table, scene=self.scene, rays=(o, d), samples=samples, n=n, layout=1, n_dev=n_dev, out=out)
+
+    def _density_stream(self, o, d, samples, n, return_feat: bool = False, n_dev=None, x_unit=None):
+        feat = self._hash_features(o, d, samples, n, x_unit=x_unit, n_dev=n_dev)
         if self.cfg.mlp_kernels == "x":
             _, sigma, _, _ = ops.mlp_fwd_x(self.field.mlp, self.field.C, self._xmode(), feat, self.scene, rays=(o, d),
                                            samples=samples, n=n, density_only=True, act=self._act_code, n_dev=n_dev)
@@ -400,8 +413,7 @@
         chunks = min(self.cfg.fwd_chunks, pk.n >> 20) if pk.n >= (1 << 23) else 1
         if self.cfg.mlp_kernels == "x" and chunks > 1 and pk.feat is None and pk.n_dev is None:
             return self._field_forward_chunked(o, d, pk, save, chunks)
-        feat = pk.feat if pk.feat is not None else \
-            ops.hashgrid_fwd(f.grid, f.table, scene=self.scene, rays=(o, d), samples=samples, n=pk.n, layout=1, n_dev=pk.n_dev)
+        feat = pk.feat if pk.feat is not None else self._hash_features(o, d, samples, pk.n, x_unit=pk.x_unit, n_dev=pk.n_dev)
         if self.cfg.mlp_kernels == "x":
             rgb, sigma, base, acts = ops.mlp_fwd_x(f.mlp, f.C, self._xmode(), feat, self.scene, rays=(o, d), samples=samples,
                                                    n=pk.n, save=save, save_acts=self._save_acts(), act=self._act_code, n_dev=pk.n_dev)
@@ -440,7 +452,7 @@
             smp = (pk.ray_indices[lo:hi], pk.t_starts[lo:hi], pk.t_ends[lo:hi])
             fk = feat[b0 * ops.FRAG_FLOATS_PER_BLOCK: b1 * ops.FRAG_FLOATS_PER_BLOCK]
             with torch.cuda.stream(s_enc):
-                ops.hashgrid_fwd(f.grid, f.table, scene=self.scene, rays=(o, d), samples=smp, n=hi - lo, layout=1, out=fk)
+                self._hash_features(o, d, smp, hi - lo, x_unit=None if pk.x_unit is None else pk.x_unit[lo:hi], out=fk)
                 ev = torch.cuda.Event()
                 ev.record(s_enc)
             with torch.cuda.stream(s_mlp):
diff --git a/robust_e_nerf_amd/ops.py b/robust_e_nerf_amd/ops.py
--- a/robust_e_nerf_amd/ops.py
+++ b/robust_e_nerf_amd/ops.py
@@ -244,7 +244,7 @@
 
 
 def ray_march_write(o, d, t_min, t_max, jitter, roi, res, binary, ct, step, cone, mode, n_uniform,
-                    offsets, n_total: int, out=None, counts=None, cache=None):
+                    offsets, n_total: int, out=None, counts=None, cache=None, unit_scene: Optional[SceneDesc] = None):
     n = o.shape[0]
     if out is None:
         ri = torch.empty(n_total, device=o.device, dtype=torch.int32)
@@ -252,17 +252,31 @@
         te = torch.empty(n_total, device=o.device, dtype=torch.float32)
     else:
         ri, ts, te = out
+    xu = torch.empty(n_total, 3, device=o.device, dtype=torch.float32) if unit_scene is not None else None
+    ret = (ri, ts, te) if xu is None else (ri, ts, te, xu)
     if n_total == 0:
-        return ri, ts, te
+        return ret
     roi_c = (ctypes.c_float * 6)(*[float(v) for v in roi])
     res_c = (ctypes.c_int32 * 3)(*[int(v) for v in res])
-    check(_lib.load().ren_ray_march(_ptr(o), _ptr(d), _ptr(t_min), _ptr(t_max), _ptr(jitter), n, roi_c, res_c,
-                                    _ptr(binary, (torch.uint8, torch.bool)), ct, _f(step), _f(cone), mode, n_uniform,
-                                    _ptr(offsets, torch.int64), _ptr(counts, torch.int32), _ptr(ri), _ptr(ts), _ptr(te),
-                                    _ptr(cache, torch.float32) if counts is not None else None,
-                                    0 if (cache is None or counts is None) else cache.shape[1], _stream()),
-          "ren_ray_march(write)")
-    return ri, ts, te
+    args = (_ptr(o), _ptr(d), _ptr(t_min), _ptr(t_max), _ptr(jitter), n, roi_c, res_c,
+            _ptr(binary, (torch.uint8, torch.bool)), ct, _f(step), _f(cone), mode, n_uniform,
+            _ptr(offsets, torch.int64), _ptr(counts, torch.int32), _ptr(ri), _ptr(ts), _ptr(te),
+            _ptr(cache, torch.float32) if counts is not None else None,
+            0 if (cache is None or counts is None) else cache.shape[1])
+    if xu is None:
+        check(_lib.load().ren_ray_march(*args, _stream()), "ren_ray_march(write)")
+    else:
+        check(_lib.load().ren_ray_march_unit(*args, ctypes.byref(unit_scene), _ptr(xu), _stream()), "ren_ray_march_unit")
+    return ret
+
+
+def unit_positions(scene: SceneDesc, rays, samples, n: int, n_dev=None, out=None):
+    (o, d), (ri, ts, te) = rays, samples
+    if out is None:
+        out = torch.empty(n, 3, device=o.device, dtype=torch.float32)
+    check(_lib.load().ren_unit_positions(ctypes.byref(scene), _ptr(o), _ptr(d), _ptr(ri, torch.int32), _ptr(ts), _ptr(te), n,
+                                         _ptr(out, torch.float32), _ptr(n_dev, torch.int64), _stream()), "ren_unit_positions")
+    return out
 
 
 def count_guard(counts, total, capacity: int, n_out, stats=None, counts_also=None):
@@ -297,11 +311,18 @@
     return keep, kept
 
 
-def compact_samples(offsets, counts, new_offsets, keep, ts, te, n_new: int):
+def compact_samples(offsets, counts, new_offsets, keep, ts, te, n_new: int, x_unit=None):
     n_rays = counts.shape[0]
     ri2 = torch.empty(n_new, device=ts.device, dtype=torch.int32)
     ts2 = torch.empty(n_new, device=ts.device, dtype=torch.float32)
     te2 = torch.empty(n_new, device=ts.device, dtype=torch.float32)
+    if x_unit is not None:
+        xu2 = torch.empty(n_new, 3, device=ts.device, dtype=torch.float32)
+        if n_new > 0:
+            check(_lib.load().ren_compact_samples_unit(_ptr(offsets), _ptr(counts), _ptr(new_offsets), n_rays, _ptr(keep),
+                                                       _ptr(ts), _ptr(te), _ptr(x_unit, torch.float32), _ptr(ri2), _ptr(ts2),
+                                                       _ptr(te2), _ptr(xu2), _stream()), "ren_compact_samples_unit")
+        return ri2, ts2, te2, xu2
     if n_new == 0:
         return ri2, ts2, te2
     check(_lib.load().ren_compact_samples(_ptr(offsets), _ptr(counts), _ptr(new_offsets), n_rays, _ptr(keep),
```

Result: faster. 6.230 million rays/s, median of 6 (+1.3%).
